# HoangChuongNguyen/ibgs

Measured on AMD Instinct MI355X. Metric: train-step fps (fwd+bwd raster) @1080p, 1M Gaussians, higher is better.
Workload: dtype f32

## Files before the change

ibgs_amd/_build.py:

```python
import os
import subprocess
import sys
from concurrent.futures import ThreadPoolExecutor

HERE = os.path.dirname(os.path.abspath(__file__))
CSRC = os.path.join(HERE, "csrc")
OBJ = os.path.join(CSRC, "_obj")
LIB = os.path.join(HERE, "libibgs_rast.so")
SOURCES = ["api", "preprocess", "scan_sort", "binning", "render_fwd", "render_bwd", "preprocess_bwd", "knn", "adam", "compact", "deterministic", "loss", "depth_normal", "activate"]
EXTRA = {
    "preprocess": ["-ffp-contract=off"],
    "render_fwd": ["-fno-slp-vectorize"],
    "render_bwd": ["-fno-slp-vectorize", "-fno-signed-zeros"],
}
ARCH = "gfx950"


def _hipcc():
    for c in (os.environ.get("HIPCC"), "/opt/rocm/bin/hipcc", "hipcc"):
        if c and (os.path.isabs(c) and os.path.exists(c) or not os.path.isabs(c)):
            return c
    return "hipcc"


def _newest_dep():
    deps = [os.path.join(CSRC, f) for f in os.listdir(CSRC) if f.endswith((".h", ".hip"))]
    deps.append(os.path.join(HERE, "..", "include", "ibgs_rast.h"))
    return max(os.path.getmtime(d) for d in deps)


def _code_only(text):
    import re
    text = re.sub(r"/\*.*?\*/", "", text, flags=re.S)
    text = re.sub(r"//[^\n]*", "", text)
    return "\n".join(l.rstrip() for l in text.split("\n") if l.strip())


def csrc_sha():
    import hashlib
    h = hashlib.sha1()
    for f in sorted(os.listdir(CSRC)):
        if f.endswith((".hip", ".h")):
            h.update(f.encode())
            h.update(_code_only(open(os.path.join(CSRC, f), "r").read()).encode())
    h.update(_code_only(open(os.path.join(HERE, "..", "include", "ibgs_rast.h"), "r").read()).encode())
    return h.hexdigest()[:12]


KERNEL_TU = (("render_fwd", "render_fwd"), ("pack_rgba", "render_fwd"), ("render_bwd", "render_bwd"), ("geo_window", "render_bwd"), ("tile_order", "render_bwd"),
             ("preprocess_bwd", "preprocess_bwd"), ("sh_grad", "preprocess_bwd"), ("preprocess_kernel", "preprocess"), ("sh_color", "preprocess"), ("mark_visible", "preprocess"),
             ("onesweep", "scan_sort"), ("radix", "scan_sort"), ("scan_", "scan_sort"), ("cell_", "binning"), ("expand_", "binning"), ("tile_ranges", "binning"),
             ("rendered_note", "api"), ("l1_", "loss"), ("depth_normal", "depth_normal"), ("activate_", "activate"), ("adam", "adam"), ("compact", "compact"), ("det_", "deterministic"), ("knn", "knn"))


def tu_of(kernel_name):
    for sub, tu in KERNEL_TU:
        if sub in kernel_name:
            return tu
    return None


def tu_shas():
    import hashlib
    hdr = hashlib.sha1()
    for f in sorted(os.listdir(CSRC)):
        if f.endswith(".h"):
            hdr.update(f.encode()); hdr.update(_code_only(open(os.path.join(CSRC, f), "r").read()).encode())
    hdr.update(_code_only(open(os.path.join(HERE, "..", "include", "ibgs_rast.h"), "r").read()).encode())
    out = {}
    for name in SOURCES:
        h = hdr.copy()
        h.update(_code_only(open(os.path.join(CSRC, name + ".hip"), "r").read()).encode())
        h.update(" ".join(EXTRA.get(name, [])).encode())
        out[name] = h.hexdigest()[:12]
    return out


def needs_build():
    if not os.path.exists(LIB):
        return True
    newest = _newest_dep()
    objs = [os.path.join(OBJ, n + ".o") for n in SOURCES]
    return any((not os.path.exists(o)) or os.path.getmtime(o) < newest for o in objs) or os.path.getmtime(LIB) < newest


def build(force=False, verbose=False):
    os.makedirs(OBJ, exist_ok=True)
    hipcc = _hipcc()
    hdr_time = max([os.path.getmtime(os.path.join(CSRC, f)) for f in os.listdir(CSRC) if f.endswith(".h")]
                   + [os.path.getmtime(os.path.join(HERE, "..", "include", "ibgs_rast.h"))])

    def compile_one(name):
        src = os.path.join(CSRC, name + ".hip")
        obj = os.path.join(OBJ, name + ".o")
        if (not force) and os.path.exists(obj) and os.path.getmtime(obj) >= max(os.path.getmtime(src), hdr_time):
            return obj
        cmd = [hipcc, "--offload-arch=" + ARCH, "-O3", "-fPIC", "-std=c++17", "-c", src, "-o", obj] + EXTRA.get(name, [])
        if verbose:
            print(" ".join(cmd), file=sys.stderr)
        subprocess.check_call(cmd)
        return obj

    with ThreadPoolExecutor(max_workers=4) as ex:
        objs = list(ex.map(compile_one, SOURCES))
    if force or (not os.path.exists(LIB)) or os.path.getmtime(LIB) < max(os.path.getmtime(o) for o in objs):
        cmd = [hipcc, "--offload-arch=" + ARCH, "-shared", "-fPIC", "-o", LIB] + objs
        if verbose:
            print(" ".join(cmd), file=sys.stderr)
        subprocess.check_call(cmd)
    return LIB


if __name__ == "__main__":
    print(build(force="--force" in sys.argv, verbose=True))
```

ibgs_amd/csrc/api.hip:

```cpp
#include "common.h"
#include <sched.h>
#include <time.h>
#include <string.h>
#include <cstdlib>
#include <stdlib.h>
#include <stdio.h>
#include <cstdarg>
#include <cstdio>
#include <cstring>
#include <vector>
#include <map>
#include <mutex>

namespace ibgs {

static thread_local char g_err[512] = "";
void set_error(const char* fmt, ...)
{
    va_list ap; va_start(ap, fmt);
    vsnprintf(g_err, sizeof(g_err), fmt, ap);
    va_end(ap);
}

static uint32_t higher_msb(uint32_t n)
{
    uint32_t msb = sizeof(n) * 4, step = msb;
    while (step > 1) {
        step /= 2;
        if (n >> msb) msb += step; else msb -= step;
    }
    if (n >> msb) msb++;
    return msb;
}

GeomState GeomState::carve(char* base, size_t P, size_t* total)
{
    Carver c(base);
    GeomState g;
    g.rec = c.take<float>(P * REC_FLOATS);
    g.depths = c.take<float>(P);
    g.cov3D = c.take<float>(P * 6);
    g.tiles = c.take<uint32_t>(P);
    g.fp = c.take<uint4>(P);
    g.tmask_hi = c.take<uint64_t>(P * (IBGS_CULL_WORDS - 1));
    g.fp_sorted = c.take<uint4>(P);
    g.clamped = c.take<uint8_t>(P);
    g.alive64 = c.take<uint64_t>((P + 63) / 64);
    g.tile_partial = c.take<uint32_t>((P + 63) / 64 + IBGS_MAX_VIEWS + 1);
    g.sort_key[0] = c.take<uint32_t>(P); g.sort_key[1] = c.take<uint32_t>(P);
    g.sort_val[0] = c.take<uint32_t>(P); g.sort_val[1] = c.take<uint32_t>(P);
    g.offsets = c.take<uint32_t>(P + 5);
    g.hist_elems = radix_hist_elems(P);
    g.hist = c.take<uint32_t>(g.hist_elems);
    if (total) *total = (size_t)(c.cur - reinterpret_cast<uintptr_t>(base)) + 128;
    return g;
}

ImgState ImgState::carve(char* base, int W, int H, size_t* total)
{
    Carver c(base);
    ImgState im;
    const size_t HW = (size_t)W * H;
    const size_t tiles = (size_t)((W + TILE - 1) / TILE) * ((H + TILE - 1) / TILE);
    im.ranges = c.take<uint32_t>(tiles * 2);
    im.final_T = c.take<float>(HW);
    im.n_contrib = c.take<uint32_t>(HW);
    im.sum_w = c.take<float>(HW);
    im.low_high = c.take<uint32_t>(HW * 2);
    im.valid_idx = c.take<int32_t>(HW * IBGS_MAX_SRC);
    im.valid_w = c.take<float>(HW * IBGS_MAX_SRC);
    im.meta = c.take<uint32_t>(32);
    im.slot_c = c.take<uint32_t>(HW * IBGS_MAX_BUFFER_LENGTH);
    im.tile_walked = c.take<uint32_t>(tiles * 4);
    im.tile_order = c.take<uint32_t>((tiles + ORDER_CLASSES - 1) / ORDER_CLASSES * ORDER_CLASSES);
    im.tile_risky = c.take<uint32_t>(tiles * 4);
    if (total) *total = (size_t)(c.cur - reinterpret_cast<uintptr_t>(base)) + 128;
    return im;
}

BinState BinState::carve(char* base, size_t R, int W, int H, size_t* total)
{
    Carver c(base);
    BinState b;
    const size_t gx = (size_t)((W + TILE - 1) / TILE), gy = (size_t)((H + TILE - 1) / TILE), ntiles = gx * gy;
    const size_t ncells = ((gx + BIN_CELL - 1) / BIN_CELL) * ((gy + BIN_CELL - 1) / BIN_CELL);
    b.point_list = c.take<uint32_t>(R);
    b.ccap = R;
    b.cent = c.take<uint4>(R);
    b.cnt_elems = (R / 4 > (size_t)65536 ? R / 4 : (size_t)65536) + ncells;
    b.cnt = c.take<uint32_t>(b.cnt_elems);
    b.cell_total = c.take<uint32_t>(ncells);
    b.cell_start = c.take<uint32_t>(ncells + 1);
    b.cell_chunk0 = c.take<uint32_t>(ncells + 1);
    b.chunk_cnt = c.take<uint32_t>((R / BIN_XCHUNK + ncells + 1) * 64);
    b.tile_total = c.take<uint32_t>(ntiles + 1);
    b.scan_elems = scan_scratch_elems(ntiles + 1);
    b.scan_scratch = c.take<uint32_t>(b.scan_elems);
    if (total) *total = (size_t)(c.cur - reinterpret_cast<uintptr_t>(base)) + 128;
    return b;
}

struct TimedPair { hipEvent_t a, b; int stage; };
static uint32_t g_time_mask = 0;
static std::vector<TimedPair> g_pairs;
static std::vector<hipEvent_t> g_free_events;

static hipEvent_t get_event()
{
    if (!g_free_events.empty()) { hipEvent_t e = g_free_events.back(); g_free_events.pop_back(); return e; }
    hipEvent_t e = nullptr;
    (void)hipEventCreate(&e);
    return e;
}

StageTimer::StageTimer(hipStream_t s_, int stage_) : s(s_), stage(stage_), on((g_time_mask >> stage_) & 1u)
{
    if (on) { a = get_event(); b = get_event(); (void)hipEventRecord(a, s); }
}
StageTimer::~StageTimer()
{
    if (on) { (void)hipEventRecord(b, s); g_pairs.push_back({a, b, stage}); }
}

static int stage_check(hipStream_t s, bool debug, const char* what)
{
    if (!debug) return 0;
    hipError_t e = hipStreamSynchronize(s);
    if (e == hipSuccess) e = hipGetLastError();
    if (e != hipSuccess) { set_error("stage '%s' failed: %s", what, hipGetErrorString(e)); return -IBGS_ERR_HIP; }
    return 0;
}

__global__ void __launch_bounds__(1024) rendered_note_kernel(RenderedNote n)
{
    __shared__ unsigned long long s_w[16];
    rendered_note_block<1024>(n, s_w);
}

}

using namespace ibgs;

extern "C" {

const char* ibgs_last_error(void) { return g_err; }
const char* ibgs_version(void) { return "ibgs_rast 0.1 (gfx950)"; }
void ibgs_timing_enable(uint32_t stage_mask) { g_time_mask = stage_mask; }
int32_t ibgs_timing_collect(float* ms, int32_t* launches)
{
    for (int i = 0; i < IBGS_NUM_STAGES; i++) { if (ms) ms[i] = 0.f; if (launches) launches[i] = 0; }
    for (auto& p : g_pairs) {
        float t = 0.f;
        hipError_t e = hipEventSynchronize(p.b);
        if (e == hipSuccess) e = hipEventElapsedTime(&t, p.a, p.b);
        if (e != hipSuccess) { set_error("timing collect: %s", hipGetErrorString(e)); return -IBGS_ERR_HIP; }
        if (ms) ms[p.stage] += t;
        if (launches) launches[p.stage] += 1;
        g_free_events.push_back(p.a); g_free_events.push_back(p.b);
    }
    g_pairs.clear();
    return 0;
}
size_t ibgs_sizeof_forward_args(void) { return sizeof(ibgs_forward_args); }
size_t ibgs_sizeof_backward_args(void) { return sizeof(ibgs_backward_args); }

size_t ibgs_required_geom(int32_t P) { size_t t; GeomState::carve(nullptr, (size_t)(P > 0 ? P : 0), &t); return t; }
size_t ibgs_required_img(int32_t W, int32_t H) { size_t t; ImgState::carve(nullptr, W, H, &t); return t; }
size_t ibgs_required_binning(int64_t R, int32_t W, int32_t H) { size_t t; BinState::carve(nullptr, (size_t)(R > 0 ? R : 0), W, H, &t); return t; }
size_t ibgs_required_deterministic(int64_t R, int32_t P) { size_t t; DetState::carve(nullptr, (size_t)(R > 0 ? R : 0) * 4, (size_t)(P > 0 ? P : 0), &t); return t; }
size_t ibgs_required_tex(int32_t n_src, int32_t W, int32_t H) { return (size_t)n_src * W * H * sizeof(float4) + 128; }
size_t ibgs_required_geo_table(int32_t W, int32_t H) { return geo_table_floats(W, H) * sizeof(float) + 128; }
size_t ibgs_required_geo_table_for(int32_t W, int32_t H, int32_t L)
{
    const int slots = (L >= 1 && L < IBGS_MAX_BUFFER_LENGTH) ? L + 1 : IBGS_MAX_BUFFER_LENGTH;
    return (size_t)W * H * slots * GEO_TAB_FIELDS * sizeof(float) + 128;
}
size_t ibgs_required_deterministic_for(int64_t R, int32_t P, int32_t W, int32_t H, int32_t render_geo, uint32_t flags)
{
    ibgs_backward_args a{}; a.W = W; a.H = H; a.render_geo = render_geo; a.flags = flags;
    size_t t; DetState::carve(nullptr, (size_t)(R > 0 ? R : 0) * render_backward_waves_per_tile(a), (size_t)(P > 0 ? P : 0), &t); return t;
}

#define OFF(base_struct, field) if (!strcmp(name, #field)) return (int64_t)((char*)base_struct.field - (char*)nullptr)
int64_t ibgs_geom_offset(int32_t P, const char* name)
{
    size_t t; GeomState g = GeomState::carve(nullptr, (size_t)P, &t);
    OFF(g, rec); OFF(g, depths); OFF(g, cov3D); OFF(g, tiles); OFF(g, fp); OFF(g, tmask_hi); OFF(g, clamped); OFF(g, offsets);
    if (!strcmp(name, "order")) return (int64_t)((char*)g.sort_val[0] - (char*)nullptr);
    if (!strcmp(name, "order_alt")) return (int64_t)((char*)g.sort_val[1] - (char*)nullptr);
    if (!strcmp(name, "sorted_depth_keys")) return (int64_t)((char*)g.sort_key[0] - (char*)nullptr);
    if (!strcmp(name, "sorted_depth_keys_alt")) return (int64_t)((char*)g.sort_key[1] - (char*)nullptr);
    return -1;
}
size_t ibgs_tile_order_slots(int32_t W, int32_t H)
{
    const size_t tiles = (size_t)((W + TILE - 1) / TILE) * ((H + TILE - 1) / TILE);
    return (tiles + ORDER_CLASSES - 1) / ORDER_CLASSES * ORDER_CLASSES;
}
int64_t ibgs_img_offset(int32_t W, int32_t H, const char* name)
{
    size_t t; ImgState im = ImgState::carve(nullptr, W, H, &t);
    OFF(im, ranges); OFF(im, final_T); OFF(im, n_contrib); OFF(im, sum_w); OFF(im, low_high); OFF(im, valid_idx); OFF(im, valid_w); OFF(im, slot_c); OFF(im, meta); OFF(im, tile_walked); OFF(im, tile_order); OFF(im, tile_risky);
    return -1;
}
int64_t ibgs_binning_offset(int64_t R, int32_t W, int32_t H, const char* name)
{
    size_t t; BinState b = BinState::carve(nullptr, (size_t)R, W, H, &t);
    OFF(b, point_list);
    return -1;
}
#undef OFF

struct RSlot {
    uint32_t* host; hipEvent_t ev;
    uint32_t* stats; bool stats_pending;
    bool flag_pending;
    hipStream_t last_stream;
    uint32_t seq;
};
static std::mutex g_slot_mutex;
static std::map<std::pair<int, hipStream_t>, RSlot*> g_slots;
static RSlot* rslot(hipStream_t s, bool create)
{
    int dev = 0;
    if (hipGetDevice(&dev) != hipSuccess) { set_error("hipGetDevice failed"); return nullptr; }
    std::lock_guard<std::mutex> lock(g_slot_mutex);
    auto it = g_slots.find({dev, s});
    if (it != g_slots.end()) return it->second;
    if (!create) return nullptr;
    RSlot* slot = new RSlot();
    void* p = nullptr;
    if (hipHostMalloc(&p, 64, hipHostMallocCoherent | hipHostMallocMapped) != hipSuccess) { delete slot; set_error("hipHostMalloc for the R read-back failed"); return nullptr; }
    if (hipEventCreateWithFlags(&slot->ev, hipEventDisableTiming) != hipSuccess) { (void)hipHostFree(p); delete slot; set_error("hipEventCreate failed"); return nullptr; }
    slot->host = static_cast<uint32_t*>(p);
    memset(p, 0, 64);
    slot->stats = slot->host + 8;
    slot->stats_pending = false; slot->flag_pending = false; slot->last_stream = s; slot->seq = 0;
    g_slots[{dev, s}] = slot;
    return slot;
}
static int check_sort_flag(RSlot* rs, bool wait_for_note)
{
    if (!rs || !rs->flag_pending) return 0;
    volatile uint32_t* note = rs->stats + 4;
    bool final_ = __atomic_load_n(const_cast<uint32_t*>(note), __ATOMIC_ACQUIRE) == rs->seq;
    if (!final_ && wait_for_note) {
        struct timespec t0, t1; clock_gettime(CLOCK_MONOTONIC, &t0);
        for (uint32_t spins = 1; !final_; spins++) {
            final_ = __atomic_load_n(const_cast<uint32_t*>(note), __ATOMIC_ACQUIRE) == rs->seq;
            if ((spins & 255u) == 0) {
                clock_gettime(CLOCK_MONOTONIC, &t1);
                if ((t1.tv_sec - t0.tv_sec) * 1000000000ll + (t1.tv_nsec - t0.tv_nsec) > 2000000ll) break;
            }
        }
    }
    if (*(volatile uint32_t*)(rs->stats + 3)) {
        rs->stats[3] = 0u; rs->flag_pending = false;
        set_error("depth sort: decoupled look-back timed out (the lists of this stream's last forward were mis-ordered)"); return -IBGS_ERR_HIP;
    }
    if (final_) rs->flag_pending = false;
    return 0;
}

static thread_local int64_t g_last_stats[3] = {0, -1, 0};
static thread_local RSlot* g_stats_slot = nullptr;
void ibgs_last_forward_stats(int64_t* out)
{
    if (g_stats_slot && g_stats_slot->stats_pending) {
        if (hipStreamSynchronize(g_stats_slot->last_stream) == hipSuccess) g_last_stats[1] = (int64_t)*(volatile uint32_t*)(g_stats_slot->stats + 2);
        g_stats_slot->stats_pending = false;
    }
    out[0] = g_last_stats[0]; out[1] = g_last_stats[1]; out[2] = g_last_stats[2];
}
void ibgs_debug_set_lookback_spins(uint32_t v) { radix_set_lookback_spins(v); }
int32_t ibgs_check_async(void* stream, int32_t wait)
{
    hipStream_t s = reinterpret_cast<hipStream_t>(stream);
    RSlot* rs = rslot(s, false);
    if (!rs || !rs->flag_pending) return 0;
    if (wait) IBGS_HIP(hipStreamSynchronize(s));
    return check_sort_flag(rs, false);
}

int64_t ibgs_forward(const ibgs_forward_args* ap)
{
    if (!ap) { set_error("null args"); return -IBGS_ERR_INVALID; }
    const ibgs_forward_args& a = *ap;
    hipStream_t s = reinterpret_cast<hipStream_t>(a.stream);
    const bool debug = (a.flags & IBGS_FLAG_DEBUG) != 0;
    if (a.P < 0 || a.W <= 0 || a.H <= 0) { set_error("bad sizes P=%d W=%d H=%d", a.P, a.W, a.H); return -IBGS_ERR_INVALID; }
    if (a.P == 0) return 0;
    if (!a.means3D || !a.opacities || !a.viewmatrix || !a.projmatrix || !a.campos || !a.bg || !a.radii) {
        set_error("missing required pointer"); return -IBGS_ERR_INVALID;
    }
    if ((a.shs == nullptr) == (a.colors_precomp == nullptr) && !a.render_depth_only) {
        set_error("provide exactly one of shs / colors_precomp"); return -IBGS_ERR_INVALID;
    }
    if (((a.scales == nullptr) || (a.rotations == nullptr)) == (a.cov3D_precomp == nullptr)) {
        set_error("provide exactly one of scales+rotations / cov3D_precomp"); return -IBGS_ERR_INVALID;
    }
    if (a.shs && (a.D < 0 || a.D > 3 || (a.D + 1) * (a.D + 1) > a.M)) { set_error("bad SH degree D=%d M=%d", a.D, a.M); return -IBGS_ERR_INVALID; }
    if (a.shs && a.M == 16 && (reinterpret_cast<uintptr_t>(a.shs) & 15u)) { set_error("shs (M = 16) must be 16-byte aligned"); return -IBGS_ERR_INVALID; }
    if (a.shs_rest && (!a.shs || a.M < 2 || (reinterpret_cast<uintptr_t>(a.shs_rest) & 15u) || (reinterpret_cast<uintptr_t>(a.shs) & 15u))) {
        set_error("shs_rest needs shs (the DC coefficients), M >= 2 and 16-byte aligned arrays"); return -IBGS_ERR_INVALID;
    }
    if (a.render_geo && a.render_depth_only) { set_error("render_geo together with render_depth_only is not supported"); return -IBGS_ERR_INVALID; }
    if (a.plane_mode != IBGS_PLANE_NONE) {
        if (a.all_map) { set_error("give either all_map or plane_mode, not both"); return -IBGS_ERR_INVALID; }
        if (a.plane_mode == IBGS_PLANE_LEARNT ? !a.plane_normal : (a.plane_mode != IBGS_PLANE_SMALLEST_AXIS || !a.scales || !a.rotations)) {
            set_error("plane_mode %d: plane_normal (learnt) or scales + rotations (smallest axis) required", a.plane_mode); return -IBGS_ERR_INVALID;
        }
    }
    if ((a.render_geo || a.render_depth_only) && !a.all_map && a.plane_mode == IBGS_PLANE_NONE) { set_error("all_map (or plane_mode) is required for render_geo / render_depth_only"); return -IBGS_ERR_INVALID; }
    if (a.render_geo || a.render_depth_only) {
        if (a.buffer_length < 1 || a.buffer_length > IBGS_MAX_BUFFER_LENGTH) { set_error("buffer_length %d outside 1..%d", a.buffer_length, IBGS_MAX_BUFFER_LENGTH); return -IBGS_ERR_INVALID; }
        if (!a.out_depth) { set_error("out_depth required"); return -IBGS_ERR_INVALID; }
    }
    if (a.render_geo) {
        if (a.n_src < 1 || a.n_src > IBGS_MAX_SRC) { set_error("n_src %d outside 1..%d", a.n_src, IBGS_MAX_SRC); return -IBGS_ERR_INVALID; }
        if (!a.ref_to_src || !a.src_cam_pos || !a.src_images || !a.src_depths) { set_error("source view pointers required for render_geo"); return -IBGS_ERR_INVALID; }
        if (a.flags & IBGS_FLAG_SRC_DEPTH_SLOTS) {
            for (int m = 0; m < a.n_src; m++) if (a.src_depth_slot[m] < 0) { set_error("src_depth_slot[%d] = %d is negative", m, a.src_depth_slot[m]); return -IBGS_ERR_INVALID; }
        }
        if (!a.out_normal || !a.out_cam_feat || !a.out_warped || !a.out_min_depth_diff || !a.out_camera_ray || !a.out_mask) { set_error("geo outputs required"); return -IBGS_ERR_INVALID; }
        if (!a.tex || a.tex_bytes < ibgs_required_tex(a.n_src, a.W, a.H)) { set_error("tex scratch too small"); return -IBGS_ERR_ALLOC; }
    }
    if (!a.render_depth_only && !a.out_color) { set_error("out_color required"); return -IBGS_ERR_INVALID; }
    const int nv = a.n_views > 1 ? a.n_views : 1;
    if (nv > 1) {
        if (nv > IBGS_MAX_VIEWS || !a.render_depth_only || a.plane_mode == IBGS_PLANE_NONE) {
            set_error("n_views = %d needs render_depth_only, plane_mode != 0 and n_views <= %d", a.n_views, IBGS_MAX_VIEWS); return -IBGS_ERR_INVALID;
        }
        if ((int64_t)nv * a.P > 0x7FFFFFFF) { set_error("n_views x P too large"); return -IBGS_ERR_INVALID; }
    }
    const int Pn = nv * a.P;
    const int Hn = nv > 1 ? nv * TILE * ((a.H + TILE - 1) / TILE) : a.H;
    if (!a.geom || a.geom_bytes < ibgs_required_geom(Pn)) { set_error("geom arena too small"); return -IBGS_ERR_ALLOC; }
    if (!a.img || a.img_bytes < ibgs_required_img(a.W, Hn)) { set_error("img arena too small"); return -IBGS_ERR_ALLOC; }
    if (!a.binning_alloc) { set_error("binning_alloc callback required"); return -IBGS_ERR_INVALID; }

    int rc;
    GeomState g = GeomState::carve(a.geom, (size_t)Pn, nullptr);
    ImgState im = ImgState::carve(a.img, a.W, Hn, nullptr);
    const int gx = (a.W + TILE - 1) / TILE, gy = nv * ((a.H + TILE - 1) / TILE);

    const bool deferred = a.rendered_hint > 0 && !debug;
    const size_t nwaves = (size_t)nv * (((size_t)a.P + 63) / 64);
    RSlot* rs = rslot(s, true);
    if (!rs) return -IBGS_ERR_HIP;
    uint32_t ticket = 0;
    { StageTimer t(s, IBGS_STAGE_PREPROCESS);
      if ((rc = launch_preprocess(s, a, g, deferred ? 1 : 0))) return rc;
      if (deferred) {
          ticket = ++rs->seq;
          const RenderedNote note{g.tile_partial, (uint32_t)nwaves, ticket, rs->host};
          if ((rc = launch_preprocess(s, a, g, 2, &note)) < 0) return rc;
          if (rc == 0) { hipLaunchKernelGGL(rendered_note_kernel, dim3(1), dim3(1024), 0, s, note); IBGS_HIP(hipGetLastError()); }
      }
    }
    if ((rc = stage_check(s, debug, "preprocess"))) return rc;
    { StageTimer t(s, IBGS_STAGE_DEPTH_SORT);
      if ((rc = radix_sort_pairs(s, g.sort_key, g.sort_val, (size_t)Pn, 32, g.hist, g.hist_elems, deferred ? g.tile_partial + nwaves : g.offsets + Pn + 1,
                                 g.offsets + Pn + 3, true, g.offsets + Pn + 4))) return rc; }
    if ((rc = stage_check(s, debug, "depth sort"))) return rc;
    { StageTimer t(s, IBGS_STAGE_SCAN);
      if (!deferred && (rc = exclusive_scan_u32(s, g.tiles, g.offsets, (size_t)Pn, g.hist, g.hist_elems, true))) return rc; }
    auto exact_R = [&](int64_t* R_out) -> int {
        IBGS_HIP(hipMemcpyAsync(rs->host, g.offsets + Pn, 2 * sizeof(uint32_t), hipMemcpyDeviceToHost, s));
        IBGS_HIP(hipEventRecord(rs->ev, s));
        IBGS_HIP(hipEventSynchronize(rs->ev));
        if (rs->host[1]) { set_error("depth sort: decoupled look-back timed out (lists would be mis-ordered)"); return -IBGS_ERR_HIP; }
        *R_out = (int64_t)rs->host[0];
        return 0;
    };
    int64_t R = 0, cap = 0;
    if (deferred) cap = a.rendered_hint < (int64_t)0xFFFF0000ll ? a.rendered_hint : (int64_t)0xFFFF0000ll;
    else { if ((rc = exact_R(&R))) return rc; cap = R; }

    auto tail = [&](int64_t n, bool read_back) -> int {
        int rc;
        const size_t need = ibgs_required_binning(n, a.W, Hn);
        char* bin_mem = (read_back && a.binning && a.binning_bytes >= need) ? a.binning : a.binning_alloc(need, a.binning_user);
        if (!bin_mem) { set_error("binning_alloc returned NULL for R=%lld", (long long)n); return -IBGS_ERR_ALLOC; }
        BinState b = BinState::carve(bin_mem, (size_t)n, a.W, Hn, nullptr);
        { StageTimer t(s, IBGS_STAGE_EMIT);
          if ((rc = launch_binning(s, Pn, n, gx, gy, g, b, im.ranges, a.tile_order_hint, im.meta, nv, read_back ? g.tile_partial + nwaves : nullptr, read_back ? rs->stats : nullptr, ticket))) return rc; }
        if (read_back) { rs->flag_pending = true; rs->last_stream = s; }
        { StageTimer t(s, IBGS_STAGE_TILE_SORT); if ((rc = launch_binning_scatter(s, n, gx, gy, b))) return rc; }
        if ((rc = stage_check(s, debug, "binning"))) return rc;
        const float4* rgba = nullptr;
        if (a.render_geo) {
            float4* t = reinterpret_cast<float4*>((reinterpret_cast<uintptr_t>(a.tex) + 127) & ~uintptr_t(127));
            if (!(a.flags & IBGS_FLAG_TEX_PACKED) && (rc = launch_pack_rgba(s, a.src_images, t, a.W, a.H, a.n_src))) return rc;
            rgba = t;
        }
        { StageTimer t(s, IBGS_STAGE_RENDER_FWD); if ((rc = launch_render_forward(s, a, g, b, im, rgba))) return rc; }
        return stage_check(s, debug, "render");
    };
    const bool prev_pending = rs->flag_pending;
    if ((rc = tail(cap, deferred))) return rc;
    g_last_stats[1] = -1; g_last_stats[2] = 0;
    g_stats_slot = rs; rs->stats_pending = false;
    if (deferred) {
        {
            volatile uint32_t* tk = rs->host + 2;
            const uint32_t want = ticket;
            uint64_t spins = 0;
            struct timespec t0; bool timed = false;
            while (__atomic_load_n(const_cast<uint32_t*>(tk), __ATOMIC_ACQUIRE) != want) {
                if (++spins > 4000) {
                    if (!timed) { clock_gettime(CLOCK_MONOTONIC, &t0); timed = true; }
                    sched_yield();
                    if ((spins & 1023) == 0) {
                        struct timespec t1; clock_gettime(CLOCK_MONOTONIC, &t1);
                        if (t1.tv_sec - t0.tv_sec > 5) {
                            if (hipStreamQuery(s) == hipErrorNotReady) { t0 = t1; continue; }
                            IBGS_HIP(hipStreamSynchronize(s));
                            if (*tk == want) break;
                            set_error("ibgs_forward: the device never reported R (ticket %u, last seen %u)", want, *tk); return -IBGS_ERR_HIP;
                        }
                    }
                }
            }
        }
        if (prev_pending && *(volatile uint32_t*)(rs->stats + 3)) {
            rs->stats[3] = 0u;
            set_error("depth sort of the previous forward: decoupled look-back timed out (its lists were mis-ordered)"); return -IBGS_ERR_HIP;
        }
        const uint64_t sum = (uint64_t)rs->host[0] | ((uint64_t)rs->host[1] << 32);
        R = (int64_t)sum;
        if (R > cap) {
            g_last_stats[2] = 1;
            IBGS_HIP(hipStreamSynchronize(s));
            if ((rc = check_sort_flag(rs, false))) return rc;
            if ((rc = tail(R, false))) return rc;
        } else rs->stats_pending = true;
    }
    g_last_stats[0] = R;
    return R;
}

int32_t ibgs_backward(const ibgs_backward_args* ap)
{
    if (!ap) { set_error("null args"); return -IBGS_ERR_INVALID; }
    const ibgs_backward_args& a = *ap;
    hipStream_t s = reinterpret_cast<hipStream_t>(a.stream);
    const bool debug = (a.flags & IBGS_FLAG_DEBUG) != 0;
    if (a.P <= 0) return 0;
    RSlot* rs = rslot(s, false);
    { int frc = check_sort_flag(rs, false); if (frc) return frc; }
    if (!a.geom || !a.img || (!a.binning && a.R > 0)) { set_error("backward needs the forward's arenas"); return -IBGS_ERR_INVALID; }
    if (!a.grad_acc) { set_error("grad_acc scratch required"); return -IBGS_ERR_INVALID; }
    if (!a.dL_dmean2D || (!a.dL_dmean2D_abs && !(a.flags & IBGS_FLAG_NO_ABS_GRAD)) || !a.dL_dopacity || !a.dL_dmean3D) {
        set_error("missing gradient output"); return -IBGS_ERR_INVALID;
    }
    if (a.shs && !a.dL_dsh && !(a.flags & IBGS_FLAG_SH_FACTORED)) { set_error("dL_dsh required"); return -IBGS_ERR_INVALID; }
    if (a.shs_rest && (!a.shs || a.M < 2 || (!(a.flags & IBGS_FLAG_SH_FACTORED) && !a.dL_dsh_rest)
                       || ((reinterpret_cast<uintptr_t>(a.shs_rest) | reinterpret_cast<uintptr_t>(a.shs) | reinterpret_cast<uintptr_t>(a.dL_dsh_rest) | reinterpret_cast<uintptr_t>(a.dL_dsh)) & 15u))) {
        set_error("shs_rest needs shs, M >= 2, dL_dsh_rest and 16-byte aligned arrays"); return -IBGS_ERR_INVALID;
    }
    if (a.shs && a.M == 16 && ((reinterpret_cast<uintptr_t>(a.shs) & 15u) || (a.dL_dsh && (reinterpret_cast<uintptr_t>(a.dL_dsh) & 15u)))) {
        set_error("shs / dL_dsh (M = 16) must be 16-byte aligned"); return -IBGS_ERR_INVALID;
    }
    if (!a.dL_dcolors && (!a.shs || (a.flags & IBGS_FLAG_SH_FACTORED))) { set_error("dL_dcolors required (precomputed colours, or IBGS_FLAG_SH_FACTORED)"); return -IBGS_ERR_INVALID; }
    if (!a.dL_dcov3D && a.cov3D_precomp) { set_error("dL_dcov3D required with cov3D_precomp"); return -IBGS_ERR_INVALID; }
    if (a.scales && (!a.dL_dscale || !a.dL_drot)) { set_error("dL_dscale / dL_drot required"); return -IBGS_ERR_INVALID; }
    if (a.render_geo) {
        if (a.plane_mode == IBGS_PLANE_NONE ? (!a.all_map || !a.dL_dall_map)
                                            : (a.plane_mode == IBGS_PLANE_LEARNT ? (!a.plane_normal || !a.dL_dplane_normal)
                                                                                 : (a.plane_mode != IBGS_PLANE_SMALLEST_AXIS || !a.scales || !a.rotations))) {
            set_error("geo backward: plane inputs / gradient outputs missing"); return -IBGS_ERR_INVALID;
        }
        if (!a.out_depth || !a.out_warped || !a.ref_to_src || !a.src_images) { set_error("geo backward inputs missing"); return -IBGS_ERR_INVALID; }
        if (!a.tex || a.tex_bytes < ibgs_required_tex(a.n_src, a.W, a.H)) { set_error("tex scratch too small"); return -IBGS_ERR_ALLOC; }
        if (!a.geo_table || a.geo_table_bytes < (a.buffer_length > 0 ? ibgs_required_geo_table_for(a.W, a.H, a.buffer_length) : ibgs_required_geo_table(a.W, a.H))) { set_error("geo_table scratch too small"); return -IBGS_ERR_ALLOC; }
    }
    int rc;
    GeomState g = GeomState::carve(a.geom, (size_t)a.P, nullptr);
    ImgState im = ImgState::carve(a.img, a.W, a.H, nullptr);
    BinState b = BinState::carve(a.binning, (size_t)a.R, a.W, a.H, nullptr);
    const float4* rgba = nullptr;
    float* geo_tab = nullptr;
    if (a.render_geo) {
        float4* t = reinterpret_cast<float4*>((reinterpret_cast<uintptr_t>(a.tex) + 127) & ~uintptr_t(127));
        const bool window = a.dL_ddepth || a.dL_dwarped;
        if (window && !(a.flags & IBGS_FLAG_TEX_PACKED) && (rc = launch_pack_rgba(s, a.src_images, t, a.W, a.H, a.n_src))) return rc;
        rgba = t;
        geo_tab = reinterpret_cast<float*>((reinterpret_cast<uintptr_t>(a.geo_table) + 127) & ~uintptr_t(127));
    }
    if (a.R > 0) {
        const bool det = (a.flags & IBGS_FLAG_DETERMINISTIC) != 0;
        DetState ds{};
        int ipt = 1;
        if (det) {
            if (!a.det_scratch || a.det_scratch_bytes < ibgs_required_deterministic_for(a.R, a.P, a.W, a.H, a.render_geo, a.flags)) { set_error("det_scratch too small"); return -IBGS_ERR_ALLOC; }
            ipt = render_backward_waves_per_tile(a);
            ds = DetState::carve(a.det_scratch, (size_t)a.R * ipt, (size_t)a.P, nullptr);
            if ((rc = launch_det_prepare(s, ds, (size_t)a.R * ipt))) return rc;
        }
        if ((rc = launch_render_backward(s, a, g, b, im, rgba, det ? ds.slab : nullptr, geo_tab))) return rc;
        if (det) { StageTimer t(s, IBGS_STAGE_TILE_ORDER); if ((rc = launch_det_reduce(s, ds, b.point_list, (size_t)a.R, ipt, a.P, a.grad_acc, g.offsets + a.P))) return rc; }
        if ((rc = stage_check(s, debug, "render backward"))) return rc;
    }
    { StageTimer t(s, IBGS_STAGE_PREPROCESS_BWD); if ((rc = launch_preprocess_backward(s, a, g))) return rc; }
    if ((rc = stage_check(s, debug, "preprocess backward"))) return rc;
    return check_sort_flag(rs, true);
}

int32_t ibgs_sh_grad_from_views(void* stream, int32_t P, int32_t D, int32_t M, int32_t n_views, const float* means3D,
                                const float* camposes, const float* dcolor, int64_t view_stride, float* dL_dsh)
{
    if (view_stride == 0) view_stride = (int64_t)P * 3;
    if (view_stride < (int64_t)P * 3) { set_error("view_stride smaller than P x 3"); return -IBGS_ERR_INVALID; }
    if (P <= 0 || M <= 0) return 0;
    if (D < 0 || D > 3 || (D + 1) * (D + 1) > M || n_views < 0) { set_error("bad SH degree / view count"); return -IBGS_ERR_INVALID; }
    if (!means3D || !dL_dsh || (n_views > 0 && (!camposes || !dcolor))) { set_error("null pointer"); return -IBGS_ERR_INVALID; }
    return launch_sh_grad_from_views(reinterpret_cast<hipStream_t>(stream), P, D, M, n_views, means3D, camposes, dcolor, (size_t)view_stride, dL_dsh);
}

int32_t ibgs_mark_visible(void* stream, int32_t P, const float* means3D, const float* viewmatrix,
                          const float* projmatrix, uint8_t* present)
{
    (void)projmatrix;
    if (P <= 0) return 0;
    if (!means3D || !viewmatrix || !present) { set_error("null pointer"); return -IBGS_ERR_INVALID; }
    return launch_mark_visible(reinterpret_cast<hipStream_t>(stream), P, means3D, viewmatrix, present);
}

}
```

ibgs_amd/csrc/common.h:

```cpp
#pragma once
#include <hip/hip_runtime.h>
#include <stdint.h>
#include <stddef.h>
#include <stdlib.h>
#include "../../include/ibgs_rast.h"

namespace ibgs {

constexpr int TILE = IBGS_TILE;
constexpr int WAVE = 64;
constexpr int REC_FLOATS = 16;
constexpr int GACC_FLOATS = 16;

constexpr int IBGS_CULL_WORDS = 4;
constexpr int IBGS_CULL_MAX_TILES = 64 * IBGS_CULL_WORDS;

enum RecField { R_X = 0, R_Y = 1, R_OP = 2, R_PAD0 = 3, R_CA = 4, R_CB = 5, R_CC = 6, R_DIST = 7,
                R_R = 8, R_G = 9, R_B = 10, R_PAD1 = 11, R_NX = 12, R_NY = 13, R_NZ = 14, R_PAD2 = 15 };

enum GaccField { G_SX = 0, G_SY = 1, G_AX = 2, G_AY = 3, G_SXX = 4, G_SXY = 5, G_SYY = 6, G_S0 = 7,
                 G_R = 8, G_G = 9, G_B = 10, G_NX = 11, G_NY = 12, G_NZ = 13, G_DIST = 14, G_PAD = 15 };

struct Carver {
    uintptr_t cur;
    explicit Carver(char* base) : cur(reinterpret_cast<uintptr_t>(base)) {}
    template <typename T> T* take(size_t count) {
        cur = (cur + 127) & ~uintptr_t(127);
        T* p = reinterpret_cast<T*>(cur);
        cur += count * sizeof(T);
        return p;
    }
};

struct GeomState {
    float* rec;
    float* depths;
    float* cov3D;
    uint32_t* tiles;
    uint4* fp;
    uint64_t* tmask_hi;
    uint4* fp_sorted;
    uint8_t* clamped;
    uint64_t* alive64;
    uint32_t* tile_partial;
    uint32_t* sort_key[2];
    uint32_t* sort_val[2];
    uint32_t* offsets;
    uint32_t* hist;
    size_t hist_elems;
    static GeomState carve(char* base, size_t P, size_t* total);
};

struct ImgState {
    uint32_t* ranges;
    float* final_T;
    uint32_t* n_contrib;
    float* sum_w;
    uint32_t* low_high;
    int32_t* valid_idx;
    float* valid_w;
    uint32_t* meta;
    uint32_t* slot_c;
    uint32_t* tile_walked;
    uint32_t* tile_order;
    uint32_t* tile_risky;
    static ImgState carve(char* base, int W, int H, size_t* total);
};

constexpr int BIN_CELL = 8;
constexpr int BIN_XCHUNK = 256;

struct BinState {
    uint32_t* point_list;
    uint4* cent;
    uint32_t* cnt;
    size_t cnt_elems;
    uint32_t* cell_total;
    uint32_t* cell_start;
    uint32_t* cell_chunk0;
    uint32_t* chunk_cnt;
    uint32_t* tile_total;
    uint32_t* scan_scratch; size_t scan_elems;
    size_t ccap;
    static BinState carve(char* base, size_t R, int W, int H, size_t* total);
};

constexpr float EXP2_SCALE = 0.5f * 1.4426950408889634f;
constexpr float EXP2_UNSCALE = 1.0f / EXP2_SCALE;
constexpr float ALPHA_SKIP_E = 7.9943533f;
__device__ __forceinline__ void stage_for_exp2(float4& pos_opacity_quad, float4& conic_quad)
{
    conic_quad.x *= EXP2_SCALE; conic_quad.y *= EXP2_SCALE; conic_quad.z *= EXP2_SCALE;
    pos_opacity_quad.z = -__builtin_amdgcn_logf(pos_opacity_quad.z);
}

constexpr float POWER_RISK = 0.99999f;
constexpr float LOG2_E = 1.4426950408889634f;
__device__ __forceinline__ bool conic_is_risky(float a, float b, float c) { return b * b > POWER_RISK * (a * c); }
constexpr float BLEND_REF_POWER_RISK = 0.999f;
__device__ __forceinline__ bool conic_takes_ref_power(float a, float b, float c) { return b * b > BLEND_REF_POWER_RISK * (a * c); }
__device__ __forceinline__ float ref_power_E(float dx, float dy, float a, float b, float c, float neg_log2_opacity)
{
#pragma clang fp contract(off)
    const float power = -0.5f * (a * dx * dx + c * dy * dy) - b * dx * dy;
    return power > 0.0f ? __builtin_inff() : fmaf(-power, LOG2_E, neg_log2_opacity);
}

__device__ __forceinline__ float ln_portable(float x)
{
#pragma clang fp contract(off)
    uint32_t u = __float_as_uint(x);
    const int e = (int)(u >> 23) - 127;
    u = (u & 0x007FFFFFu) | 0x3F800000u;
    const float m = __uint_as_float(u);
    const float s = (m - 1.0f) / (m + 1.0f), z = s * s;
    const float poly = 1.0f + z * (0.33333334f + z * (0.2f + z * (0.14285715f + z * 0.11111111f)));
    return (float)e * 0.6931472f + 2.0f * s * poly;
}
__device__ __forceinline__ float cull_qmax(float o)
{
#pragma clang fp contract(off)
    return 2.0f * ln_portable(255.0f * o) * 1.001f + 0.001f;
}
struct CullRows { float px, py, B, det, invA, aq, ymax, ystar; int x0, x1; };
__device__ __forceinline__ void cull_rows_setup(CullRows& j, float px, float py, float A, float B, float C, float det, float qmax, int x0, int x1)
{
#pragma clang fp contract(off)
    j.px = px; j.py = py; j.B = B; j.det = det; j.x0 = x0; j.x1 = x1;
    j.invA = 1.0f / A; j.aq = A * qmax;
    j.ymax = sqrtf(j.aq / det); j.ystar = -B * sqrtf(qmax / (C * det));
}
__device__ __forceinline__ void cull_rows_setup_conic(CullRows& j, float px, float py, float A, float B, float C, float qmax, int x0, int x1)
{
#pragma clang fp contract(off)
    const float det = A * C - B * B;
    cull_rows_setup(j, px, py, A, B, C, det, qmax, x0, x1);
}
__device__ __forceinline__ bool cull_row_run(const CullRows& j, int ty, int& t0, int& t1)
{
#pragma clang fp contract(off)
    const float Y0 = (float)(ty * 16) - j.py, Y1 = Y0 + 15.0f;
    const float yb0 = Y0 > -j.ymax ? Y0 : -j.ymax, yb1 = Y1 < j.ymax ? Y1 : j.ymax;
    if (yb0 > yb1) return false;
    const float yu = __builtin_amdgcn_fmed3f(j.ystar, yb0, yb1), yl = __builtin_amdgcn_fmed3f(-j.ystar, yb0, yb1);
    const float eu = j.aq - j.det * yu * yu, el = j.aq - j.det * yl * yl;
    const float du = eu > 0.0f ? eu : 0.0f, dl = el > 0.0f ? el : 0.0f;
    const float xhi = (-j.B * yu + sqrtf(du)) * j.invA, xlo = (-j.B * yl - sqrtf(dl)) * j.invA;
    t0 = (int)ceilf((xlo - 0.01f + j.px - 15.0f) / 16.0f); t1 = (int)floorf((xhi + 0.01f + j.px) / 16.0f);
    t0 = max(t0, j.x0); t1 = min(t1, j.x1 - 1);
    return t1 >= t0;
}

#ifdef IBGS_TRACE_WAVES
constexpr int IBGS_TRACE_MAX = 32768;
#define IBGS_TRACE_BEGIN() const unsigned long long ibgs_trace_t0_ = __builtin_amdgcn_s_memrealtime()
#define IBGS_TRACE_END(buf)                                                                                         \
    do {                                                                                                            \
        const unsigned long long t1_ = __builtin_amdgcn_s_memrealtime();                                            \
        if (threadIdx.x == 0 && blockIdx.x < (unsigned)IBGS_TRACE_MAX)                                              \
            (buf)[blockIdx.x] = make_uint4(__builtin_amdgcn_s_getreg((31 << 11) | 4), __builtin_amdgcn_s_getreg((31 << 11) | 20), \
                                           (uint32_t)ibgs_trace_t0_, (uint32_t)t1_);                                \
    } while (0)
#else
#define IBGS_TRACE_BEGIN() do { } while (0)
#define IBGS_TRACE_END(buf) do { } while (0)
#endif

#ifdef IBGS_COUNT_LANES
#define IBGS_LANES_DECL() unsigned long long ibgs_lc_[4] = {0ull, 0ull, 0ull, 0ull}
#define IBGS_LANES_ADD(i, n) ibgs_lc_[i] += (unsigned long long)(n)
#define IBGS_LANES_FLUSH(buf) do { if (threadIdx.x == 0) { for (int i_ = 0; i_ < 4; i_++) atomicAdd(&(buf)[i_], ibgs_lc_[i_]); } } while (0)
#else
#define IBGS_LANES_DECL() do { } while (0)
#define IBGS_LANES_ADD(i, n) do { } while (0)
#define IBGS_LANES_FLUSH(buf) do { } while (0)
#endif

void set_error(const char* fmt, ...);
#define IBGS_HIP(expr)                                                                    \
    do {                                                                                  \
        hipError_t e_ = (expr);                                                           \
        if (e_ != hipSuccess) {                                                           \
            ::ibgs::set_error("%s failed: %s (%s:%d)", #expr, hipGetErrorString(e_), __FILE__, __LINE__); \
            return -IBGS_ERR_HIP;                                                         \
        }                                                                                 \
    } while (0)

struct StageTimer {
    hipStream_t s; hipEvent_t a = nullptr, b = nullptr; int stage; bool on;
    StageTimer(hipStream_t s_, int stage_);
    ~StageTimer();
};

struct Cam {
    const float* vm;
    const float* pm;
    const float* campos;
    const float* bg;
    float tanfovx, tanfovy, fx, fy;
    int W, H, gx, gy;
};
inline Cam make_cam(const float* vm, const float* pm, const float* campos, const float* bg,
                    float tanfovx, float tanfovy, int W, int H)
{
    Cam c;
    c.vm = vm; c.pm = pm; c.campos = campos; c.bg = bg;
    c.tanfovx = tanfovx; c.tanfovy = tanfovy;
    c.fy = H / (2.0f * tanfovy); c.fx = W / (2.0f * tanfovx);
    c.W = W; c.H = H; c.gx = (W + TILE - 1) / TILE; c.gy = (H + TILE - 1) / TILE;
    return c;
}


struct PlaneEval {
    float n[3];
    float ncam[3];
    float dist;
    float flip;
    float sgn;
    float inv_len;
    int axis;
};

__device__ __forceinline__ PlaneEval plane_eval(int mode, const float* __restrict__ raw_n, const float* __restrict__ raw_off,
                                                const float* __restrict__ scales, const float* __restrict__ rot, int i,
                                                float mx, float my, float mz, const float* __restrict__ campos,
                                                const float* __restrict__ vm)
{
    PlaneEval e;
    float off = 0.f;
    e.inv_len = 1.f; e.axis = 0;
    if (mode == IBGS_PLANE_LEARNT) {
        const float a = raw_n[3 * i], b = raw_n[3 * i + 1], c = raw_n[3 * i + 2];
        const float len = sqrtf(a * a + b * b + c * c);
        e.inv_len = 1.0f / len;
        e.n[0] = a / len; e.n[1] = b / len; e.n[2] = c / len;
        off = raw_off ? raw_off[i] : 0.f;
    } else {
        const float s0 = scales[3 * i], s1 = scales[3 * i + 1], s2 = scales[3 * i + 2];
        int k = 0; float sm = s0;
        if (s1 < sm) { sm = s1; k = 1; }
        if (s2 < sm) { sm = s2; k = 2; }
        e.axis = k;
        const float r = rot[4 * i], x = rot[4 * i + 1], y = rot[4 * i + 2], z = rot[4 * i + 3];
        if (k == 0)      { e.n[0] = 1.f - 2.f * (y * y + z * z); e.n[1] = 2.f * (x * y + r * z);       e.n[2] = 2.f * (x * z - r * y); }
        else if (k == 1) { e.n[0] = 2.f * (x * y - r * z);       e.n[1] = 1.f - 2.f * (x * x + z * z); e.n[2] = 2.f * (y * z + r * x); }
        else             { e.n[0] = 2.f * (x * z + r * y);       e.n[1] = 2.f * (y * z - r * x);       e.n[2] = 1.f - 2.f * (x * x + y * y); }
    }
    const float tc = e.n[0] * (campos[0] - mx) + e.n[1] * (campos[1] - my) + e.n[2] * (campos[2] - mz);
    e.flip = (tc < 0.0f) ? -1.f : 1.f;
    e.n[0] *= e.flip; e.n[1] *= e.flip; e.n[2] *= e.flip; off *= e.flip;
#pragma unroll
    for (int j = 0; j < 3; j++) e.ncam[j] = e.n[0] * vm[j] + e.n[1] * vm[4 + j] + e.n[2] * vm[8 + j];
    float gd = -(e.n[0] * mx + e.n[1] * my + e.n[2] * mz);
    if (mode == IBGS_PLANE_LEARNT) gd += off;
    const float sd = gd - (e.ncam[0] * vm[12] + e.ncam[1] * vm[13] + e.ncam[2] * vm[14]);
    e.sgn = sd > 0.f ? 1.f : (sd < 0.f ? -1.f : 0.f);
    e.dist = fabsf(sd);
    return e;
}

enum { TMAP_RR = 0, TMAP_GROUP = 1, TMAP_BLOCK = 2 };
struct TileMap { int mode, g, bx, by; };
inline int tile_map_grid(const TileMap& m, int gx, int gy, int ipt)
{
    if (m.mode == TMAP_BLOCK) {
        const int nb = ((gx + m.bx - 1) / m.bx) * ((gy + m.by - 1) / m.by);
        return ((nb + 7) / 8) * 8 * m.bx * m.by * ipt;
    }
    const int g = m.mode == TMAP_GROUP ? m.g : 1;
    return ((gx * gy * ipt + 8 * g - 1) / (8 * g)) * 8 * g;
}
__device__ __forceinline__ bool tile_map_item(const TileMap& m, int b, int gx, int gy, int ipt, int& tile, int& sub)
{
    const int xcd = b & 7, idx = b >> 3;
    if (m.mode == TMAP_BLOCK) {
        const int per = m.bx * m.by * ipt;
        const int blk = (idx / per) * 8 + xcd, within = idx % per;
        const int nbx = (gx + m.bx - 1) / m.bx;
        const int t = within / ipt;
        const int tx = (blk % nbx) * m.bx + t % m.bx, ty = (blk / nbx) * m.by + t / m.bx;
        sub = within % ipt;
        tile = ty * gx + tx;
        return tx < gx && ty < gy;
    }
    int item = b;
    if (m.mode == TMAP_GROUP) item = ((idx / m.g) * 8 + xcd) * m.g + idx % m.g;
    tile = item / ipt; sub = item % ipt;
    return item < gx * gy * ipt;
}

__device__ __forceinline__ bool hybrid_split(uint32_t work, unsigned long long total, uint32_t theta_pct)
{
    return (unsigned long long)work * 1024ull * 100ull > total * theta_pct;
}
constexpr uint32_t ORDER_SPLIT_BIT = 0x80000000u;
__device__ __forceinline__ bool hybrid_item(int b, int grid1, const uint32_t* __restrict__ order, int& tile, int& sub, bool& split)
{
    const int idx = (b - grid1) >> 3;
    const int slot = b < grid1 ? b : (idx / 3) * 8 + (b & 7);
    sub = b < grid1 ? 0 : idx % 3 + 1;
    const uint32_t t = order[slot];
    split = (t & ORDER_SPLIT_BIT) != 0u;
    tile = (int)(t & ~ORDER_SPLIT_BIT);
    return t != 0xFFFFFFFFu;
}
__device__ __forceinline__ bool hybrid_item_mapped(const TileMap& m, int b, int grid1, int gx, int gy, int& tile, int& sub)
{
    if (b < grid1) { const bool ok = tile_map_item(m, b, gx, gy, 1, tile, sub); sub = 0; return ok; }
    const bool ok = tile_map_item(m, b - grid1, gx, gy, 3, tile, sub);
    sub += 1;
    return ok;
}
constexpr int HYBRID_THETA = 50;
constexpr int HYBRID_MIN_TILES = 768;
constexpr int hybrid_max_tiles() { return 4096; }
constexpr int hybrid_theta() { return HYBRID_THETA; }

struct RenderedNote { const uint32_t* partial; uint32_t nwords; uint32_t ticket; uint32_t* host; };
template <int NT>
__device__ __forceinline__ void rendered_note_block(const RenderedNote& n, unsigned long long* s_w )
{
    unsigned long long sum = 0;
    for (uint32_t i = threadIdx.x; i < n.nwords; i += NT) sum += n.partial[i];
    for (int d = 32; d >= 1; d >>= 1) sum += __shfl_xor(sum, d, 64);
    if ((threadIdx.x & 63) == 0) s_w[threadIdx.x >> 6] = sum;
    __syncthreads();
    if (threadIdx.x == 0) {
        unsigned long long t = 0;
        for (int w = 0; w < NT / 64; w++) t += s_w[w];
        volatile uint32_t* host_words = n.host;
        host_words[0] = (uint32_t)t; host_words[1] = (uint32_t)(t >> 32);
        __threadfence_system();
        __hip_atomic_store(n.host + 2, n.ticket, __ATOMIC_RELEASE, __HIP_MEMORY_SCOPE_SYSTEM);
    }
}
int launch_preprocess(hipStream_t s, const ibgs_forward_args& a, const GeomState& g, int phase = 0, const RenderedNote* note = nullptr);
int launch_mark_visible(hipStream_t s, int P, const float* means3D, const float* vm, uint8_t* present);

size_t radix_hist_elems(size_t n);
int radix_sort_pairs(hipStream_t s, uint32_t* keys[2], uint32_t* vals[2], size_t n, int nbits,
                     uint32_t* hist, size_t hist_elems, uint32_t* err_dev = nullptr, uint32_t* kept_dev = nullptr, bool scratch_is_zero = false,
                     uint32_t* result_alt = nullptr);
size_t radix_zero_elems(size_t n, int nbits);
int exclusive_scan_u32(hipStream_t s, const uint32_t* in, uint32_t* out, size_t n, uint32_t* scratch,
                       size_t scratch_elems, bool with_total);
size_t scan_scratch_elems(size_t n);
void radix_set_onesweep(bool on);
void radix_set_lookback_spins(uint32_t v);

int launch_binning(hipStream_t s, int P, int64_t cap, int gx, int gy, const GeomState& g, const BinState& b, uint32_t* ranges,
                   const uint32_t* order_hint = nullptr, uint32_t* meta = nullptr ,
                   int n_views = 1 ,
                   const uint32_t* sort_flag = nullptr, uint32_t* host_note = nullptr ,
                   uint32_t note_ticket = 0 );
constexpr int ORDER_CLASSES = 1024;
int launch_binning_scatter(hipStream_t s, int64_t cap, int gx, int gy, const BinState& b);

int launch_pack_rgba(hipStream_t s, const float* src, float4* dst, int W, int H, int n);
constexpr int GEO_TAB_FIELDS = 6;
inline size_t geo_table_floats(int W, int H) { return (size_t)W * H * IBGS_MAX_BUFFER_LENGTH * GEO_TAB_FIELDS; }
int launch_render_forward(hipStream_t s, const ibgs_forward_args& a, const GeomState& g, const BinState& b,
                          const ImgState& im, const float4* src_rgba);
int launch_render_backward(hipStream_t s, const ibgs_backward_args& a, const GeomState& g, const BinState& b,
                           const ImgState& im, const float4* src_rgba, float* slab = nullptr, float* geo_tab = nullptr);
int launch_preprocess_backward(hipStream_t s, const ibgs_backward_args& a, const GeomState& g);

struct DetState {
    float* slab;
    uint32_t* keys[2];
    uint32_t* vals[2];
    uint32_t* seg;
    uint32_t* hist; size_t hist_elems;
    static DetState carve(char* base, size_t rows, size_t P, size_t* total);
};
int render_backward_waves_per_tile(const ibgs_backward_args& a);
int render_backward_ref_arith(uint32_t flags);
int launch_det_prepare(hipStream_t s, const DetState& d, size_t rows);
int launch_det_reduce(hipStream_t s, const DetState& d, const uint32_t* point_list, size_t R, int ipt, int P, float* gacc, const uint32_t* listed );
int launch_sh_grad_from_views(hipStream_t s, int P, int D, int M, int n_views, const float* means3D, const float* camposes,
                              const float* dcolor, size_t view_stride, float* dL_dsh);

__device__ __forceinline__ uint32_t pack_rect(int lo, int hi) { return (uint32_t)lo | ((uint32_t)hi << 16); }

}
```

ibgs_amd/csrc/preprocess.hip:

```cpp
#include "common.h"
#include <stdlib.h>

namespace ibgs {

__constant__ float kC0 = 0.28209479177387814f;
__constant__ float kC1 = 0.4886025119029199f;
__constant__ float kC2[5] = {1.0925484305920792f, -1.0925484305920792f, 0.31539156525252005f,
                             -1.0925484305920792f, 0.5462742152960396f};
__constant__ float kC3[7] = {-0.5900435899266435f, 2.890611442640554f, -0.4570457994644658f,
                             0.3731763325901154f, -0.4570457994644658f, 1.445305721320277f,
                             -0.5900435899266435f};

struct PreParams {
    int P, D, M;
    const float* means3D; const float* scales; const float* rotations; const float* opacities;
    const float* shs; const float* shs_rest;
    const float* cov3D_precomp; const float* colors_precomp; const float* all_map;
    const float* plane_normal; const float* plane_offset; int plane_mode;
    int inst0;
    int tile_row0;
    float scale_modifier;
    int depth_only;
    int32_t* radii;
    float* rec; float* depths; float* cov3D; uint32_t* tiles; uint4* fp; uint64_t* tmask_hi; uint8_t* clamped;
    uint64_t* alive64;
    uint32_t* sort_key; uint32_t* sort_val;
    int cull;
    uint32_t* zero_a; uint32_t zero_a_n; uint32_t* zero_b; uint32_t zero_b_n;
    RenderedNote note;
    uint32_t* tile_partial; int partial0; int partial_err;
};

__device__ __forceinline__ float ndc_to_pix(float v, int S)
{
    return (float)((((double)v + 1.0) * S - 1.0) * 0.5);
}

__device__ __forceinline__ int clampi(int v, int lo, int hi) { return min(hi, max(lo, v)); }

struct CullJob { CullRows rows; int y0, w, h; };
enum { CULL_NONE = 0, CULL_AABB = 1, CULL_ROWS = 2 };

__device__ __forceinline__ int cull_setup(float px, float py, float sxx, float syy, float A, float B, float C, float o,
                                          int& x0, int& y0, int& x1, int& y1, CullJob& j)
{
    if (conic_is_risky(A, B, C)) return CULL_AABB;
    const float x255 = 255.0f * o;
    if (!(x255 >= 1.0f)) { x1 = x0; y1 = y0; return CULL_NONE; }
    const float qmax = cull_qmax(o);
    const float hx = sqrtf(qmax * sxx), hy = sqrtf(qmax * syy);
    int tx0 = (int)ceilf((px - hx - 15.0f) / 16.0f), tx1 = (int)floorf((px + hx) / 16.0f) + 1;
    int ty0 = (int)ceilf((py - hy - 15.0f) / 16.0f), ty1 = (int)floorf((py + hy) / 16.0f) + 1;
    tx0 = max(tx0, x0); tx1 = min(tx1, x1); ty0 = max(ty0, y0); ty1 = min(ty1, y1);
    if (tx1 <= tx0 || ty1 <= ty0) { x1 = x0; y1 = y0; return CULL_NONE; }
    x0 = tx0; x1 = tx1; y0 = ty0; y1 = ty1;
    const float det = A * C - B * B;
    if (!(A > 0.0f) || !(C > 0.0f) || !(det > 0.0f)) return CULL_AABB;
    cull_rows_setup(j.rows, px, py, A, B, C, det, qmax, tx0, tx1);
    j.y0 = ty0; j.w = tx1 - tx0; j.h = ty1 - ty0;
    return CULL_ROWS;
}

__device__ __forceinline__ void set_run(uint64_t (&m)[IBGS_CULL_WORDS], int start, int len)
{
#pragma unroll
    for (int k = 0; k < IBGS_CULL_WORDS; k++) {
        const int lo = max(start, 64 * k), hi = min(start + len, 64 * k + 64);
        if (lo < hi) m[k] |= ((hi - lo == 64) ? ~0ull : ((1ull << (hi - lo)) - 1ull)) << (lo - 64 * k);
    }
}

constexpr int CULL_COOP_ROWS = 16;
__device__ __forceinline__ void park_job(float4* stage_row, const CullJob& j)
{
    stage_row[0] = make_float4(j.rows.px, j.rows.py, j.rows.B, j.rows.det);
    stage_row[1] = make_float4(j.rows.invA, j.rows.aq, j.rows.ymax, j.rows.ystar);
    stage_row[2] = make_float4(__uint_as_float((uint32_t)j.rows.x0 | ((uint32_t)j.rows.x1 << 16)), __uint_as_float((uint32_t)j.y0 | ((uint32_t)j.h << 16)), 0.f, 0.f);
    stage_row[3] = make_float4(0.f, 0.f, 0.f, 0.f);
    stage_row[4] = make_float4(0.f, 0.f, 0.f, 0.f);
}
__device__ __forceinline__ void fetch_job(const float4* stage_row, CullJob& j)
{
    const float4 q0 = stage_row[0], q1 = stage_row[1], q2 = stage_row[2];
    j.rows.px = q0.x; j.rows.py = q0.y; j.rows.B = q0.z; j.rows.det = q0.w;
    j.rows.invA = q1.x; j.rows.aq = q1.y; j.rows.ymax = q1.z; j.rows.ystar = q1.w;
    const uint32_t xs = __float_as_uint(q2.x), ys = __float_as_uint(q2.y);
    j.rows.x0 = (int)(xs & 0xFFFFu); j.rows.x1 = (int)(xs >> 16);
    j.y0 = (int)(ys & 0xFFFFu); j.h = (int)(ys >> 16); j.w = j.rows.x1 - j.rows.x0;
}
__device__ __forceinline__ void wave_flat_rows(float4* stage, int rows, int lane)
{
    uint32_t* words = reinterpret_cast<uint32_t*>(stage);
    int incl = rows;
#pragma unroll
    for (int d = 1; d < 64; d <<= 1) { const int o = __shfl_up(incl, d, 64); if (lane >= d) incl += o; }
    const int total = __builtin_amdgcn_readlane(incl, 63);
    for (int base = 0; base < total; base += 64) {
        const int item = base + lane;
        int lo = 0;
#pragma unroll
        for (int step = 32; step >= 1; step >>= 1) { const int v = __shfl(incl, lo + step - 1, 64); if (v <= item) lo += step; }
        const int owner = min(lo, 63);
        const int r = item - (__shfl(incl, owner, 64) - __shfl(rows, owner, 64));
        if (item < total) {
            CullJob u;
            fetch_job(stage + owner * 5, u);
            int t0, t1;
            if (cull_row_run(u.rows, u.y0 + r, t0, t1)) {
                uint32_t* ow = words + owner * 20;
                atomicAdd(ow + 10, (uint32_t)(t1 - t0 + 1));
                if (u.w * u.h <= IBGS_CULL_MAX_TILES) {
                    const int s0 = r * u.w + (t0 - u.rows.x0), e0 = s0 + (t1 - t0 + 1);
                    for (int k = s0 >> 5; k <= (e0 - 1) >> 5; k++) {
                        const int lo_b = max(s0, 32 * k) - 32 * k, hi_b = min(e0, 32 * k + 32) - 32 * k;
                        atomicOr(ow + 12 + k, ((hi_b - lo_b == 32) ? ~0u : ((1u << (hi_b - lo_b)) - 1u)) << lo_b);
                    }
                }
            }
        }
    }
}

template <bool WITH_SH>
__global__ void __launch_bounds__(256, 4) preprocess_kernel(PreParams p, Cam cam)
{
    __shared__ float4 s_stage_all[4][64 * 5];
    float4* s_stage = s_stage_all[threadIdx.x >> 6];
    const int gi = blockIdx.x * blockDim.x + threadIdx.x;
    for (uint32_t z = (uint32_t)gi; z < p.zero_a_n; z += gridDim.x * blockDim.x) p.zero_a[z] = 0u;
    if ((uint32_t)gi < p.zero_b_n) p.zero_b[gi] = 0u;
    const bool valid = gi < p.P;
    const int i = valid ? gi : p.P - 1;

    float rec[REC_FLOATS];
#pragma unroll
    for (int k = 0; k < REC_FLOATS; k++) rec[k] = 0.f;
    int radius = 0; uint32_t ntiles = 0; float depth = 0.f; uint8_t clampbits = 0;
    float c6loc[6] = {0, 0, 0, 0, 0, 0};

    const float px3 = p.means3D[3 * i], py3 = p.means3D[3 * i + 1], pz3 = p.means3D[3 * i + 2];
    const float* __restrict__ vm = cam.vm; const float* __restrict__ pm = cam.pm;
    const float hx = pm[0] * px3 + pm[4] * py3 + pm[8] * pz3 + pm[12];
    const float hy = pm[1] * px3 + pm[5] * py3 + pm[9] * pz3 + pm[13];
    const float hw = pm[3] * px3 + pm[7] * py3 + pm[11] * pz3 + pm[15];
    const float pw = 1.0f / (hw + 0.0000001f);
    const float zview = vm[2] * px3 + vm[6] * py3 + vm[10] * pz3 + vm[14];

    bool alive = zview > 0.2f;
    float ca = 0.f, cb = 0.f, cc = 0.f, det_inv = 0.f, pxs = 0.f, pys = 0.f;
    int x0 = 0, y0 = 0, x1 = 0, y1 = 0;
    int walk_rows = 0;
    bool full_mask = false;
    const int lane = threadIdx.x & 63;
    if (alive) {
        if (p.cov3D_precomp) {
#pragma unroll
            for (int k = 0; k < 6; k++) c6loc[k] = p.cov3D_precomp[6 * i + k];
        } else {
            const float r = p.rotations[4 * i], x = p.rotations[4 * i + 1], y = p.rotations[4 * i + 2], z = p.rotations[4 * i + 3];
            float R[3][3];
            R[0][0] = 1.f - 2.f * (y * y + z * z); R[0][1] = 2.f * (x * y - r * z);       R[0][2] = 2.f * (x * z + r * y);
            R[1][0] = 2.f * (x * y + r * z);       R[1][1] = 1.f - 2.f * (x * x + z * z); R[1][2] = 2.f * (y * z - r * x);
            R[2][0] = 2.f * (x * z - r * y);       R[2][1] = 2.f * (y * z + r * x);       R[2][2] = 1.f - 2.f * (x * x + y * y);
            const float sv[3] = {p.scale_modifier * p.scales[3 * i], p.scale_modifier * p.scales[3 * i + 1],
                                 p.scale_modifier * p.scales[3 * i + 2]};
            float Mm[3][3];
#pragma unroll
            for (int a = 0; a < 3; a++)
#pragma unroll
                for (int b = 0; b < 3; b++) Mm[a][b] = sv[a] * R[b][a];
#define SIG(a, b) (Mm[0][a] * Mm[0][b] + Mm[1][a] * Mm[1][b] + Mm[2][a] * Mm[2][b])
            c6loc[0] = SIG(0, 0); c6loc[1] = SIG(0, 1); c6loc[2] = SIG(0, 2);
            c6loc[3] = SIG(1, 1); c6loc[4] = SIG(1, 2); c6loc[5] = SIG(2, 2);
#undef SIG
        }
        float t0 = vm[0] * px3 + vm[4] * py3 + vm[8] * pz3 + vm[12];
        float t1 = vm[1] * px3 + vm[5] * py3 + vm[9] * pz3 + vm[13];
        const float t2 = vm[2] * px3 + vm[6] * py3 + vm[10] * pz3 + vm[14];
        const float limx = 1.3f * cam.tanfovx, limy = 1.3f * cam.tanfovy;
        const float txtz = t0 / t2, tytz = t1 / t2;
        t0 = fminf(limx, fmaxf(-limx, txtz)) * t2;
        t1 = fminf(limy, fmaxf(-limy, tytz)) * t2;
        const float j00 = cam.fx / t2, j02 = -(cam.fx * t0) / (t2 * t2);
        const float j11 = cam.fy / t2, j12 = -(cam.fy * t1) / (t2 * t2);
        float A[2][3];
#pragma unroll
        for (int r = 0; r < 3; r++) {
            const float rv0 = vm[4 * r + 0], rv1 = vm[4 * r + 1], rv2 = vm[4 * r + 2];
            A[0][r] = rv0 * j00 + rv1 * 0.0f + rv2 * j02;
            A[1][r] = rv0 * 0.0f + rv1 * j11 + rv2 * j12;
        }
        const float S[3][3] = {{c6loc[0], c6loc[1], c6loc[2]}, {c6loc[1], c6loc[3], c6loc[4]}, {c6loc[2], c6loc[4], c6loc[5]}};
        float SA[2][3];
#pragma unroll
        for (int a = 0; a < 2; a++)
#pragma unroll
            for (int r = 0; r < 3; r++) SA[a][r] = S[r][0] * A[a][0] + S[r][1] * A[a][1] + S[r][2] * A[a][2];
        ca = A[0][0] * SA[0][0] + A[0][1] * SA[0][1] + A[0][2] * SA[0][2] + 0.3f;
        cb = A[0][0] * SA[1][0] + A[0][1] * SA[1][1] + A[0][2] * SA[1][2];
        cc = A[1][0] * SA[1][0] + A[1][1] * SA[1][1] + A[1][2] * SA[1][2] + 0.3f;
        const float det = ca * cc - cb * cb;
        alive = (det != 0.0f);
        if (alive) {
            det_inv = 1.f / det;
            const float mid = 0.5f * (ca + cc);
            const float disc = sqrtf(fmaxf(0.1f, mid * mid - det));
            const float lam1 = mid + disc, lam2 = mid - disc;
            const float my_radius = ceilf(3.f * sqrtf(fmaxf(lam1, lam2)));
            pxs = ndc_to_pix(hx * pw, cam.W); pys = ndc_to_pix(hy * pw, cam.H);
            const int rad = (int)my_radius;
            x0 = clampi((int)((pxs - rad) / TILE), 0, cam.gx);
            y0 = clampi((int)((pys - rad) / TILE), 0, cam.gy);
            x1 = clampi((int)((pxs + rad + TILE - 1) / TILE), 0, cam.gx);
            y1 = clampi((int)((pys + rad + TILE - 1) / TILE), 0, cam.gy);
            alive = ((x1 - x0) * (y1 - y0)) != 0;
            if (alive) {
                radius = rad; ntiles = (uint32_t)((x1 - x0) * (y1 - y0));
                full_mask = true;
                if (p.cull) {
                    CullJob job;
                    const int cull_mode = cull_setup(pxs, pys, ca, cc, cc * det_inv, -cb * det_inv, ca * det_inv, p.opacities[i], x0, y0, x1, y1, job);
                    if (cull_mode == CULL_NONE) { ntiles = 0; full_mask = false; }
                    else if (cull_mode == CULL_AABB) ntiles = (uint32_t)((x1 - x0) * (y1 - y0));
                    else {
                        full_mask = false;
                        walk_rows = job.h;
                        park_job(s_stage + lane * 5, job);
                    }
                }
            }
        }
    }
    if (p.cull) {
        const bool tall = walk_rows > CULL_COOP_ROWS;
        if (__ballot(walk_rows != 0) != 0ull) {
            wave_flat_rows(s_stage, tall ? 0 : walk_rows, lane);
            uint64_t todo = __ballot(tall);
            while (todo != 0ull) {
                const int g = __builtin_ctzll(todo);
                todo &= todo - 1ull;
                CullJob u;
                fetch_job(s_stage + g * 5, u);
                const bool masked = u.w * u.h <= IBGS_CULL_MAX_TILES;
                uint64_t m[IBGS_CULL_WORDS] = {0, 0, 0, 0};
                uint32_t cnt = 0;
                for (int r = lane; r < u.h; r += 64) {
                    int t0, t1;
                    if (!cull_row_run(u.rows, u.y0 + r, t0, t1)) continue;
                    if (masked) set_run(m, r * u.w + (t0 - u.rows.x0), t1 - t0 + 1);
                    cnt += (uint32_t)(t1 - t0 + 1);
                }
#pragma unroll
                for (int d = 32; d >= 1; d >>= 1) cnt += (uint32_t)__shfl_xor((int)cnt, d, 64);
                uint32_t* ow = reinterpret_cast<uint32_t*>(s_stage) + g * 20;
                if (masked) {
#pragma unroll
                    for (int k = 0; k < IBGS_CULL_WORDS; k++) {
                        uint32_t lo = (uint32_t)m[k], hi = (uint32_t)(m[k] >> 32);
#pragma unroll
                        for (int d = 32; d >= 1; d >>= 1) { lo |= (uint32_t)__shfl_xor((int)lo, d, 64); hi |= (uint32_t)__shfl_xor((int)hi, d, 64); }
                        if (lane == 0) { ow[12 + 2 * k] = lo; ow[13 + 2 * k] = hi; }
                    }
                }
                if (lane == 0) ow[10] = cnt;
            }
        }
    }
    {
        uint64_t tmask[IBGS_CULL_WORDS];
        const uint32_t* ow = reinterpret_cast<const uint32_t*>(s_stage) + lane * 20;
#pragma unroll
        for (int k = 0; k < IBGS_CULL_WORDS; k++) tmask[k] = walk_rows != 0 ? (((uint64_t)ow[13 + 2 * k] << 32) | ow[12 + 2 * k]) : (full_mask ? ~0ull : 0ull);
        if (walk_rows != 0) ntiles = ow[10];
        uint32_t rx = 0, ry = 0;
        bool big_rect = false;
        if (alive) {
            big_rect = (x1 - x0) * (y1 - y0) > 64 && (x1 - x0) * (y1 - y0) <= IBGS_CULL_MAX_TILES;
            rx = pack_rect(x0, x1); ry = pack_rect(y0 + (uint32_t)p.tile_row0, y1 + (uint32_t)p.tile_row0);
        }
        if (valid) {
            const int o = p.inst0 + i;
            p.fp[o] = make_uint4(rx, ry, (uint32_t)tmask[0], (uint32_t)(tmask[0] >> 32));
            if (big_rect) {
#pragma unroll
                for (int k = 1; k < IBGS_CULL_WORDS; k++) p.tmask_hi[(size_t)o * (IBGS_CULL_WORDS - 1) + (k - 1)] = tmask[k];
            }
        }
    }
    if (alive) {
        depth = zview;
        rec[R_X] = pxs; rec[R_Y] = pys; rec[R_OP] = p.opacities[i];
        rec[R_CA] = cc * det_inv; rec[R_CB] = -cb * det_inv; rec[R_CC] = ca * det_inv;
        if (p.colors_precomp) {
            rec[R_R] = p.colors_precomp[3 * i]; rec[R_G] = p.colors_precomp[3 * i + 1]; rec[R_B] = p.colors_precomp[3 * i + 2];
        } else if (WITH_SH && !p.depth_only) {
            float d0 = px3 - cam.campos[0], d1 = py3 - cam.campos[1], d2 = pz3 - cam.campos[2];
            const float len = sqrtf(d0 * d0 + d1 * d1 + d2 * d2);
            d0 /= len; d1 /= len; d2 /= len;
            float B[16];
            int nb = 1;
            B[0] = kC0;
            if (p.D > 0) {
                const float x = d0, y = d1, z = d2;
                B[1] = -kC1 * y; B[2] = kC1 * z; B[3] = -kC1 * x; nb = 4;
                if (p.D > 1) {
                    const float xx = x * x, yy = y * y, zz = z * z, xy = x * y, yz = y * z, xz = x * z;
                    B[4] = kC2[0] * xy; B[5] = kC2[1] * yz; B[6] = kC2[2] * (2.0f * zz - xx - yy);
                    B[7] = kC2[3] * xz; B[8] = kC2[4] * (xx - yy); nb = 9;
                    if (p.D > 2) {
                        B[9] = kC3[0] * y * (3.0f * xx - yy);
                        B[10] = kC3[1] * xy * z;
                        B[11] = kC3[2] * y * (4.0f * zz - xx - yy);
                        B[12] = kC3[3] * z * (2.0f * zz - 3.0f * xx - 3.0f * yy);
                        B[13] = kC3[4] * x * (4.0f * zz - xx - yy);
                        B[14] = kC3[5] * z * (xx - yy);
                        B[15] = kC3[6] * x * (xx - 3.0f * yy);
                        nb = 16;
                    }
                }
            }
            float shv[48];
            const float* sh = p.shs + (size_t)i * p.M * 3;
            const int need = 3 * nb;
            if (p.shs_rest) {
                const float* sr = p.shs_rest + (size_t)i * (p.M - 1) * 3;
                const float* sd = p.shs + (size_t)i * 3;
#pragma unroll
                for (int k = 0; k < 48; k++) if (k < need) shv[k] = k < 3 ? sd[k] : sr[k - 3];
            } else if (p.M == 16) {
                const float4* r4 = reinterpret_cast<const float4*>(sh);
#pragma unroll
                for (int v = 0; v < 12; v++) {
                    if (4 * v < need) {
                        const float4 q = r4[v];
                        shv[4 * v] = q.x; shv[4 * v + 1] = q.y; shv[4 * v + 2] = q.z; shv[4 * v + 3] = q.w;
                    }
                }
            } else {
#pragma unroll
                for (int k = 0; k < 48; k++) if (k < need) shv[k] = sh[k];
            }
            float col[3];
#pragma unroll
            for (int ch = 0; ch < 3; ch++) col[ch] = B[0] * shv[ch];
#pragma unroll
            for (int k = 1; k < 16; k++) {
                if (k < nb) {
#pragma unroll
                    for (int ch = 0; ch < 3; ch++) col[ch] = col[ch] + B[k] * shv[3 * k + ch];
                }
            }
#pragma unroll
            for (int ch = 0; ch < 3; ch++) {
                const float v = col[ch] + 0.5f;
                if (v < 0) clampbits |= (uint8_t)(1u << ch);
                rec[R_R + ch] = fmaxf(v, 0.0f);
            }
        }
        if (p.plane_mode) {
            const PlaneEval e = plane_eval(p.plane_mode, p.plane_normal, p.plane_offset, p.scales, p.rotations, i, px3, py3, pz3, cam.campos, vm);
            rec[R_NX] = e.ncam[0]; rec[R_NY] = e.ncam[1]; rec[R_NZ] = e.ncam[2]; rec[R_DIST] = e.dist;
        } else if (p.all_map) {
            rec[R_NX] = p.all_map[5 * i]; rec[R_NY] = p.all_map[5 * i + 1]; rec[R_NZ] = p.all_map[5 * i + 2];
            rec[R_DIST] = p.all_map[5 * i + 4];
        }
    }
    if (!alive) {
#pragma unroll
        for (int k = 0; k < REC_FLOATS; k++) rec[k] = 0.f;
    }
    {
#pragma unroll
        for (int k = 0; k < 4; k++) s_stage[lane * 5 + k] = make_float4(rec[4 * k], rec[4 * k + 1], rec[4 * k + 2], rec[4 * k + 3]);
        const int first = blockIdx.x * blockDim.x + (threadIdx.x & ~63);
        const int nrow = min(64, p.P - first);
        float4* out = reinterpret_cast<float4*>(p.rec) + ((size_t)p.inst0 + first) * 4;
#pragma unroll
        for (int it = 0; it < 4; it++) {
            const int q = it * 64 + lane, row = q >> 2;
            if (row < nrow) out[q] = s_stage[row * 5 + (q & 3)];
        }
    }
    if (p.alive64) {
        const uint64_t am = __ballot(valid && alive && ntiles > 0);
        if ((threadIdx.x & 63) == 0) p.alive64[gi >> 6] = am;
    }
    {
        uint32_t tsum = valid ? ntiles : 0u;
#pragma unroll
        for (int d = 32; d >= 1; d >>= 1) tsum += (uint32_t)__shfl_xor((int)tsum, d, 64);
        if ((threadIdx.x & 63) == 0) p.tile_partial[p.partial0 + (gi >> 6)] = tsum;
        if (gi == 0) p.tile_partial[p.partial_err] = 0u;
    }
    if (!valid) return;

    const int o = p.inst0 + i;
    p.radii[o] = radius;
    p.tiles[o] = ntiles;
    p.depths[o] = depth;
    p.clamped[o] = clampbits;
    if (!p.cov3D_precomp) {
#pragma unroll
        for (int k = 0; k < 6; k++) p.cov3D[6 * o + k] = c6loc[k];
    }
    p.sort_key[o] = (alive && ntiles > 0) ? __float_as_uint(depth) : 0xFFFFFFFFu;
    p.sort_val[o] = (uint32_t)o;
}

constexpr int SHC_ROW = 52;
template <bool SPLIT>
__global__ void __launch_bounds__(256) sh_color_kernel(PreParams p, Cam cam)
{
    __shared__ float s_sh_all[4][32 * SHC_ROW];
    if (p.note.host != nullptr && blockIdx.x == 0) {
        __shared__ unsigned long long s_note[4];
        rendered_note_block<256>(p.note, s_note);
    }
    float* s_sh = s_sh_all[threadIdx.x >> 6];
    const int lane = threadIdx.x & 63;
    const int wave = blockIdx.x * 4 + (threadIdx.x >> 6);
    const int first = wave * 64;
    if (first >= p.P) return;
    const uint64_t alive_m = p.alive64[wave];
    if (alive_m == 0ull) return;
    const int i = min(first + lane, p.P - 1);
    const bool alive = (alive_m >> lane) & 1ull;
    const int D = p.D, M = p.M;
    const int nb = (D + 1) * (D + 1);
    const float px3 = p.means3D[3 * i], py3 = p.means3D[3 * i + 1], pz3 = p.means3D[3 * i + 2];
    float shv[48];
    if (SPLIT && M == 16 && first + 64 <= p.P) {
        const float4* rest4 = reinterpret_cast<const float4*>(p.shs_rest + (size_t)first * 45);
        const float4* dc4 = reinterpret_cast<const float4*>(p.shs + (size_t)first * 3);
        float4 v[12];
#pragma unroll
        for (int it = 0; it < 12; it++) {
            const int h = it / 6, qp = (it % 6) * 64 + lane;
            if (qp < 360) {
                const int ra = (4 * qp) / 45, rb = (4 * qp + 3) / 45;
                const bool need = nb > 1 && (((alive_m >> (32 * h + ra)) & 1ull) || ((alive_m >> (32 * h + rb)) & 1ull));
                v[it] = need ? rest4[360 * h + qp] : make_float4(0.f, 0.f, 0.f, 0.f);
            } else {
                const int ra = (4 * (qp - 360)) / 3, rb = (4 * (qp - 360) + 3) / 3;
                const bool need = (((alive_m >> (32 * h + ra)) & 3ull) != 0ull) || ((alive_m >> (32 * h + rb)) & 1ull);
                v[it] = need ? dc4[24 * h + (qp - 360)] : make_float4(0.f, 0.f, 0.f, 0.f);
            }
        }
        float4* s_raw = reinterpret_cast<float4*>(s_sh);
#pragma unroll
        for (int h = 0; h < 2; h++) {
#pragma unroll
            for (int it = 0; it < 6; it++) s_raw[it * 64 + lane] = v[h * 6 + it];
            if ((lane >> 5) == h) {
                const float* rr = s_sh + 45 * (lane & 31);
                const float* rd = s_sh + 1440 + 3 * (lane & 31);
                shv[0] = rd[0]; shv[1] = rd[1]; shv[2] = rd[2];
#pragma unroll
                for (int k = 0; k < 45; k++) shv[3 + k] = rr[k];
            }
        }
    } else if (SPLIT) {
        const float* sr = p.shs_rest + (size_t)i * (M - 1) * 3;
        const float* sd = p.shs + (size_t)i * 3;
#pragma unroll
        for (int k = 0; k < 48; k++) shv[k] = (alive && k < 3 * nb) ? (k < 3 ? sd[k] : sr[k - 3]) : 0.f;
    } else if (M == 16) {
        const float4* src = reinterpret_cast<const float4*>(p.shs) + (size_t)first * 12;
        const int nq = min(64, p.P - first) * 12;
        float4 v[12];
#pragma unroll
        for (int it = 0; it < 12; it++) {
            const int q = it * 64 + lane;
            const int row = q / 12, piece = q - row * 12;
            const bool ok = q < nq && ((alive_m >> row) & 1ull) && 4 * piece < 3 * nb;
            v[it] = ok ? src[q] : make_float4(0.f, 0.f, 0.f, 0.f);
        }
#pragma unroll
        for (int h = 0; h < 2; h++) {
#pragma unroll
            for (int it = 0; it < 6; it++) {
                const int q = it * 64 + lane;
                const int row = q / 12, piece = q - row * 12;
                *reinterpret_cast<float4*>(s_sh + row * SHC_ROW + piece * 4) = v[h * 6 + it];
            }
            if ((lane >> 5) == h) {
                const float4* row4 = reinterpret_cast<const float4*>(s_sh + (lane & 31) * SHC_ROW);
#pragma unroll
                for (int k = 0; k < 12; k++) { const float4 q = row4[k]; shv[4 * k] = q.x; shv[4 * k + 1] = q.y; shv[4 * k + 2] = q.z; shv[4 * k + 3] = q.w; }
            }
        }
    } else {
        const float* sh = p.shs + (size_t)i * M * 3;
#pragma unroll
        for (int k = 0; k < 48; k++) shv[k] = (alive && k < 3 * nb) ? sh[k] : 0.f;
    }
    if (!alive) return;
    float d0 = px3 - cam.campos[0], d1 = py3 - cam.campos[1], d2 = pz3 - cam.campos[2];
    const float len = sqrtf(d0 * d0 + d1 * d1 + d2 * d2);
    d0 /= len; d1 /= len; d2 /= len;
    float B[16];
    B[0] = kC0;
    if (D > 0) {
        const float x = d0, y = d1, z = d2;
        B[1] = -kC1 * y; B[2] = kC1 * z; B[3] = -kC1 * x;
        if (D > 1) {
            const float xx = x * x, yy = y * y, zz = z * z, xy = x * y, yz = y * z, xz = x * z;
            B[4] = kC2[0] * xy; B[5] = kC2[1] * yz; B[6] = kC2[2] * (2.0f * zz - xx - yy);
            B[7] = kC2[3] * xz; B[8] = kC2[4] * (xx - yy);
            if (D > 2) {
                B[9] = kC3[0] * y * (3.0f * xx - yy);
                B[10] = kC3[1] * xy * z;
                B[11] = kC3[2] * y * (4.0f * zz - xx - yy);
                B[12] = kC3[3] * z * (2.0f * zz - 3.0f * xx - 3.0f * yy);
                B[13] = kC3[4] * x * (4.0f * zz - xx - yy);
                B[14] = kC3[5] * z * (xx - yy);
                B[15] = kC3[6] * x * (xx - 3.0f * yy);
            }
        }
    }
    float col[3];
#pragma unroll
    for (int ch = 0; ch < 3; ch++) col[ch] = B[0] * shv[ch];
#pragma unroll
    for (int k = 1; k < 16; k++) {
        if (k < nb) {
#pragma unroll
            for (int ch = 0; ch < 3; ch++) col[ch] = col[ch] + B[k] * shv[3 * k + ch];
        }
    }
    const int o = p.inst0 + i;
    uint8_t clampbits = 0;
    float4 out;
    float* oc = &out.x;
#pragma unroll
    for (int ch = 0; ch < 3; ch++) {
        const float v = col[ch] + 0.5f;
        if (v < 0) clampbits |= (uint8_t)(1u << ch);
        oc[ch] = fmaxf(v, 0.0f);
    }
    out.w = 0.f;
    reinterpret_cast<float4*>(p.rec)[(size_t)o * 4 + 2] = out;
    p.clamped[o] = clampbits;
}

__global__ void __launch_bounds__(256) mark_visible_kernel(int P, const float* means3D, Cam cam, uint8_t* present)
{
    const int i = blockIdx.x * blockDim.x + threadIdx.x;
    if (i >= P) return;
    const float z = cam.vm[2] * means3D[3 * i] + cam.vm[6] * means3D[3 * i + 1] + cam.vm[10] * means3D[3 * i + 2] + cam.vm[14];
    present[i] = z > 0.2f ? 1 : 0;
}

static bool preprocess_is_split(const ibgs_forward_args& a)
{
    return a.shs && !a.colors_precomp && !a.render_depth_only;
}

int launch_preprocess(hipStream_t s, const ibgs_forward_args& a, const GeomState& g, int phase, const RenderedNote* note)
{
    PreParams p;
    p.note = RenderedNote{nullptr, 0u, 0u, nullptr};
    int carried = 0;
    p.P = a.P; p.D = a.D; p.M = a.M;
    p.means3D = a.means3D; p.scales = a.scales; p.rotations = a.rotations; p.opacities = a.opacities;
    p.shs = a.shs; p.shs_rest = a.shs_rest; p.cov3D_precomp = a.cov3D_precomp; p.colors_precomp = a.colors_precomp; p.all_map = a.all_map;
    p.plane_normal = a.plane_normal; p.plane_offset = a.plane_offset; p.plane_mode = a.plane_mode;
    p.scale_modifier = a.scale_modifier; p.depth_only = a.render_depth_only;
    p.radii = a.radii; p.rec = g.rec; p.depths = g.depths; p.cov3D = g.cov3D; p.tiles = g.tiles; p.fp = g.fp; p.tmask_hi = g.tmask_hi;
    p.clamped = g.clamped; p.sort_key = g.sort_key[0]; p.sort_val = g.sort_val[0];
    p.cull = !(a.flags & IBGS_FLAG_NO_TILE_CULL) && !(a.render_depth_only && a.buffer_length == 1);
    const int blocks = (a.P + 255) / 256;
    const int nv = a.n_views > 1 ? a.n_views : 1;
    const int gy = (a.H + TILE - 1) / TILE;
    p.zero_a = g.hist; p.zero_a_n = (uint32_t)radix_zero_elems((size_t)nv * a.P, 32);
    p.zero_b = g.offsets + (size_t)nv * a.P + 1; p.zero_b_n = 4;
    for (int v = 0; v < nv; v++) {
        p.inst0 = v * a.P; p.tile_row0 = v * gy;
        p.tile_partial = g.tile_partial; p.partial0 = v * ((a.P + 63) / 64); p.partial_err = nv * ((a.P + 63) / 64);
        const Cam cam = make_cam(a.viewmatrix + 16 * v, a.projmatrix + 16 * v, a.campos + 3 * v, a.bg,
                                 nv > 1 ? a.view_tanfovx[v] : a.tanfovx, nv > 1 ? a.view_tanfovy[v] : a.tanfovy, a.W, a.H);
        const bool split = preprocess_is_split(a);
        p.alive64 = split ? g.alive64 : nullptr;
        const bool no_sh = a.render_depth_only || a.colors_precomp || !a.shs;
        if (split) {
            if (phase != 2) hipLaunchKernelGGL(preprocess_kernel<false>, dim3(blocks), dim3(256), 0, s, p, cam);
            if (phase != 1) {
                if (note && !carried) { p.note = *note; carried = 1; } else p.note.host = nullptr;
                if (p.shs_rest) hipLaunchKernelGGL(sh_color_kernel<true>, dim3((a.P + 255) / 256), dim3(256), 0, s, p, cam);
                else hipLaunchKernelGGL(sh_color_kernel<false>, dim3((a.P + 255) / 256), dim3(256), 0, s, p, cam);
            }
        } else if (phase != 2) hipLaunchKernelGGL(preprocess_kernel<false>, dim3(blocks), dim3(256), 0, s, p, cam);
    }
    IBGS_HIP(hipGetLastError());
    return carried;
}

int launch_mark_visible(hipStream_t s, int P, const float* means3D, const float* vm, uint8_t* present)
{
    const Cam cam = make_cam(vm, nullptr, nullptr, nullptr, 1.f, 1.f, 16, 16);
    hipLaunchKernelGGL(mark_visible_kernel, dim3((P + 255) / 256), dim3(256), 0, s, P, means3D, cam, present);
    IBGS_HIP(hipGetLastError());
    return 0;
}

}
```

ibgs_amd/csrc/scan_sort.hip:

```cpp
#include "common.h"
#include <cstdlib>

namespace ibgs {

constexpr int SCAN_THREADS = 256;
constexpr int SCAN_ITEMS = 8;
constexpr int SCAN_CHUNK = SCAN_THREADS * SCAN_ITEMS;

constexpr int RS_THREADS = 256;
constexpr int RS_ITEMS = 16;
constexpr int RS_CHUNK = RS_THREADS * RS_ITEMS;
constexpr int RS_MAX_BINS = 256;

__device__ __forceinline__ uint32_t wave_inclusive_scan(uint32_t v, int lane)
{
#pragma unroll
    for (int d = 1; d < WAVE; d <<= 1) {
        const uint32_t o = __shfl_up(v, d, WAVE);
        if (lane >= d) v += o;
    }
    return v;
}

__device__ __forceinline__ uint32_t block_exclusive_scan_256(uint32_t v, uint32_t* total, uint32_t* lds_wave )
{
    const int lane = threadIdx.x & 63, wave = threadIdx.x >> 6;
    const uint32_t inc = wave_inclusive_scan(v, lane);
    if (lane == 63 && wave < 4) lds_wave[wave] = inc;
    __syncthreads();
    const uint32_t w0 = lds_wave[0], w1 = lds_wave[1], w2 = lds_wave[2], w3 = lds_wave[3];
    uint32_t base = 0;
    if (wave > 0) base += w0;
    if (wave > 1) base += w1;
    if (wave > 2) base += w2;
    *total = w0 + w1 + w2 + w3;
    __syncthreads();
    return base + inc - v;
}

__global__ void __launch_bounds__(SCAN_THREADS) scan_chunk_kernel(const uint32_t* in, uint32_t* out,
                                                                  size_t n, uint32_t* __restrict__ sums, int write_total_single)
{
    __shared__ uint32_t lds_wave[4];
    const size_t base = (size_t)blockIdx.x * SCAN_CHUNK + (size_t)threadIdx.x * SCAN_ITEMS;
    uint32_t v[SCAN_ITEMS];
    uint32_t local = 0;
#pragma unroll
    for (int k = 0; k < SCAN_ITEMS; k++) {
        v[k] = (base + k < n) ? in[base + k] : 0u;
        local += v[k];
    }
    uint32_t total;
    uint32_t pre = block_exclusive_scan_256(local, &total, lds_wave);
#pragma unroll
    for (int k = 0; k < SCAN_ITEMS; k++) {
        if (base + k < n) out[base + k] = pre;
        pre += v[k];
    }
    if (threadIdx.x == 0) {
        if (sums) sums[blockIdx.x] = total;
        if (write_total_single) out[n] = total;
    }
}

__global__ void __launch_bounds__(SCAN_THREADS) scan_add_kernel(uint32_t* __restrict__ out, size_t n, const uint32_t* __restrict__ sums,
                                                                size_t nblocks, int write_total)
{
    const size_t base = (size_t)blockIdx.x * SCAN_CHUNK + (size_t)threadIdx.x * SCAN_ITEMS;
    const uint32_t add = sums[blockIdx.x];
#pragma unroll
    for (int k = 0; k < SCAN_ITEMS; k++)
        if (base + k < n) out[base + k] += add;
    if (write_total && blockIdx.x == 0 && threadIdx.x == 0) out[n] = sums[nblocks];
}

size_t scan_scratch_elems(size_t n)
{
    size_t total = 0;
    while (n > SCAN_CHUNK) {
        n = (n + SCAN_CHUNK - 1) / SCAN_CHUNK;
        total += n + 1 + 32;
    }
    return total + 64;
}

int exclusive_scan_u32(hipStream_t s, const uint32_t* in, uint32_t* out, size_t n, uint32_t* scratch,
                       size_t scratch_elems, bool with_total)
{
    if (n == 0) {
        if (with_total) IBGS_HIP(hipMemsetAsync(out, 0, sizeof(uint32_t), s));
        return 0;
    }
    const size_t nblocks = (n + SCAN_CHUNK - 1) / SCAN_CHUNK;
    if (nblocks == 1) {
        hipLaunchKernelGGL(scan_chunk_kernel, dim3(1), dim3(SCAN_THREADS), 0, s, in, out, n, (uint32_t*)nullptr, with_total ? 1 : 0);
        IBGS_HIP(hipGetLastError());
        return 0;
    }
    if (scratch_elems < nblocks + 1) { set_error("scan scratch too small"); return -IBGS_ERR_ALLOC; }
    uint32_t* sums = scratch;
    hipLaunchKernelGGL(scan_chunk_kernel, dim3((unsigned)nblocks), dim3(SCAN_THREADS), 0, s, in, out, n, sums, 0);
    IBGS_HIP(hipGetLastError());
    const size_t used = nblocks + 1 + 32;
    int rc = exclusive_scan_u32(s, sums, sums, nblocks, scratch + used, scratch_elems > used ? scratch_elems - used : 0, true);
    if (rc) return rc;
    hipLaunchKernelGGL(scan_add_kernel, dim3((unsigned)nblocks), dim3(SCAN_THREADS), 0, s, out, n, sums, nblocks, with_total ? 1 : 0);
    IBGS_HIP(hipGetLastError());
    return 0;
}

__device__ __forceinline__ uint32_t wave_rank(uint32_t d, bool valid, int lane, uint64_t lt_mask, uint32_t* wcnt_row, unsigned long long* peer_row)
{
    uint32_t r = 0;
    if (valid) {
        atomicOr(&peer_row[d], 1ull << lane);
        const unsigned long long peers = *reinterpret_cast<volatile unsigned long long*>(&peer_row[d]);
        volatile uint32_t* wc = wcnt_row;
        const uint32_t pre = wc[d];
        r = pre + (uint32_t)__popcll(peers & lt_mask);
        if ((peers & lt_mask) == 0ull) {
            wc[d] = pre + (uint32_t)__popcll(peers);
            *reinterpret_cast<volatile unsigned long long*>(&peer_row[d]) = 0ull;
        }
    }
    return r;
}

template <typename K>
__global__ void __launch_bounds__(RS_THREADS) radix_hist_kernel(const K* __restrict__ keys, size_t n, const uint32_t* __restrict__ n_dev,
                                                                int shift, int nbins, uint32_t* __restrict__ hist, unsigned nblocks)
{
    __shared__ uint32_t h[RS_MAX_BINS];
    if (n_dev) n = min(n, (size_t)*n_dev);
    for (int k = threadIdx.x; k < nbins; k += RS_THREADS) h[k] = 0;
    __syncthreads();
    const size_t base = (size_t)blockIdx.x * RS_CHUNK;
    const uint32_t mask = (uint32_t)nbins - 1;
    const size_t i0 = base + (size_t)threadIdx.x * RS_ITEMS;
    uint32_t kv[RS_ITEMS];
    if (i0 + RS_ITEMS <= n) {
        constexpr int PER = 16 / (int)sizeof(K);
        const uint4* src = reinterpret_cast<const uint4*>(keys + i0);
#pragma unroll
        for (int v = 0; v < RS_ITEMS / PER; v++) {
            const uint4 q = src[v];
            const uint32_t w[4] = {q.x, q.y, q.z, q.w};
#pragma unroll
            for (int e = 0; e < PER; e++)
                kv[v * PER + e] = (sizeof(K) == 4) ? w[e] : ((w[e >> 1] >> ((e & 1) * 16)) & 0xFFFFu);
        }
    } else {
#pragma unroll
        for (int k = 0; k < RS_ITEMS; k++) kv[k] = (i0 + k < n) ? (uint32_t)keys[i0 + k] : 0xFFFFFFFFu;
    }
    const int nvalid = (i0 >= n) ? 0 : (int)((n - i0 < (size_t)RS_ITEMS) ? (n - i0) : (size_t)RS_ITEMS);
    uint32_t run_d = 0, run_n = 0;
#pragma unroll
    for (int k = 0; k < RS_ITEMS; k++) {
        if (k < nvalid) {
            const uint32_t d = (kv[k] >> shift) & mask;
            if (run_n != 0 && d != run_d) { atomicAdd(&h[run_d], run_n); run_n = 0; }
            run_d = d; run_n++;
        }
    }
    if (run_n != 0) atomicAdd(&h[run_d], run_n);
    __syncthreads();
    for (int k = threadIdx.x; k < nbins; k += RS_THREADS) hist[(size_t)k * nblocks + blockIdx.x] = h[k];
}

template <typename K>
__global__ void __launch_bounds__(RS_THREADS) radix_scatter_kernel(const K* __restrict__ keys_in, const uint32_t* __restrict__ vals_in,
                                                                   K* __restrict__ keys_out, uint32_t* __restrict__ vals_out,
                                                                   size_t n, const uint32_t* __restrict__ n_dev, int shift, int nbits, int nbins,
                                                                   const uint32_t* __restrict__ hist_scanned, unsigned nblocks)
{
    __shared__ uint32_t wcnt[4][RS_MAX_BINS];
    if (n_dev) n = min(n, (size_t)*n_dev);
    if ((size_t)blockIdx.x * RS_CHUNK >= n) return;
    __shared__ unsigned long long ptab[4][RS_MAX_BINS];
    __shared__ uint32_t dstart[RS_MAX_BINS];
    __shared__ uint32_t delta[RS_MAX_BINS];
    __shared__ uint32_t lds_wave[4];
    __shared__ uint32_t skey[RS_CHUNK];
    __shared__ uint32_t sval[RS_CHUNK];

    const int lane = threadIdx.x & 63, wave = threadIdx.x >> 6;
    for (int k = threadIdx.x; k < 4 * RS_MAX_BINS; k += RS_THREADS) { (&wcnt[0][0])[k] = 0; (&ptab[0][0])[k] = 0ull; }
    __syncthreads();

    const size_t base = (size_t)blockIdx.x * RS_CHUNK;
    const uint32_t mask = (uint32_t)nbins - 1;
    const uint64_t lt_mask = (lane == 0) ? 0ull : (~0ull >> (64 - lane));

    uint32_t key[RS_ITEMS], val[RS_ITEMS], rank[RS_ITEMS];
#pragma unroll
    for (int k = 0; k < RS_ITEMS; k++) {
        const size_t idx = base + (size_t)wave * (RS_ITEMS * 64) + (size_t)k * 64 + lane;
        const bool valid = idx < n;
        key[k] = valid ? (uint32_t)keys_in[idx] : 0xFFFFFFFFu;
        val[k] = valid ? vals_in[idx] : 0u;
        const uint32_t d = (key[k] >> shift) & mask;
        const uint32_t r = wave_rank(d, valid, lane, lt_mask, &wcnt[wave][0], &ptab[wave][0]);
        rank[k] = r;
    }
    __syncthreads();

    uint32_t tot = 0;
    if (threadIdx.x < nbins) {
        const uint32_t c0 = wcnt[0][threadIdx.x], c1 = wcnt[1][threadIdx.x], c2 = wcnt[2][threadIdx.x], c3 = wcnt[3][threadIdx.x];
        wcnt[0][threadIdx.x] = 0; wcnt[1][threadIdx.x] = c0; wcnt[2][threadIdx.x] = c0 + c1; wcnt[3][threadIdx.x] = c0 + c1 + c2;
        tot = c0 + c1 + c2 + c3;
    }
    uint32_t blocktotal;
    const uint32_t ds = block_exclusive_scan_256(tot, &blocktotal, lds_wave);
    if (threadIdx.x < nbins) {
        dstart[threadIdx.x] = ds;
        delta[threadIdx.x] = hist_scanned[(size_t)threadIdx.x * nblocks + blockIdx.x] - ds;
    }
    __syncthreads();

    const size_t remaining = n - base;
    const uint32_t count = remaining < (size_t)RS_CHUNK ? (uint32_t)remaining : (uint32_t)RS_CHUNK;
#pragma unroll
    for (int k = 0; k < RS_ITEMS; k++) {
        const size_t idx = base + (size_t)wave * (RS_ITEMS * 64) + (size_t)k * 64 + lane;
        if (idx < n) {
            const uint32_t d = (key[k] >> shift) & mask;
            const uint32_t lpos = dstart[d] + wcnt[wave][d] + rank[k];
            skey[lpos] = key[k];
            sval[lpos] = val[k];
        }
    }
    __syncthreads();
#pragma unroll
    for (int k = 0; k < RS_ITEMS; k++) {
        const uint32_t l = (uint32_t)k * RS_THREADS + threadIdx.x;
        if (l < count) {
            const uint32_t kk = skey[l];
            const uint32_t d = (kk >> shift) & mask;
            const uint32_t dst = l + delta[d];
            keys_out[dst] = (K)kk;
            vals_out[dst] = sval[l];
        }
    }
}


constexpr uint32_t OS_FLAG_AGG = 1u << 30, OS_FLAG_INC = 2u << 30, OS_VAL_MASK = (1u << 30) - 1u;
constexpr int OS_MAX_PASS = 4;
constexpr int OS_HIST_THREADS = 1024;
constexpr int OS_THREADS = 512, OS_WAVES = OS_THREADS / 64, OS_ITEMS = RS_CHUNK / OS_THREADS;

__global__ void __launch_bounds__(OS_HIST_THREADS) onesweep_hist_kernel(const uint32_t* __restrict__ keys, size_t n, int npass, int dbits,
                                                                   uint32_t* __restrict__ ghist ,
                                                                   int drop_max , uint32_t* __restrict__ n_kept)
{
    __shared__ uint32_t h[OS_MAX_PASS][RS_MAX_BINS];
    __shared__ uint32_t s_kept;
    for (int k = threadIdx.x; k < OS_MAX_PASS * RS_MAX_BINS; k += OS_HIST_THREADS) (&h[0][0])[k] = 0;
    if (threadIdx.x == 0) s_kept = 0;
    __syncthreads();
    const uint32_t mask = (1u << dbits) - 1u;
    const size_t stride = (size_t)gridDim.x * OS_HIST_THREADS;
    uint32_t kept = 0;
    for (size_t i = (size_t)blockIdx.x * OS_HIST_THREADS + threadIdx.x; i < n; i += stride) {
        const uint32_t k = keys[i];
        if (drop_max && k == 0xFFFFFFFFu) continue;
        kept++;
        for (int p = 0; p < npass; p++) atomicAdd(&h[p][(k >> (p * dbits)) & mask], 1u);
    }
    if (kept) atomicAdd(&s_kept, kept);
    __syncthreads();
    if (threadIdx.x == 0 && s_kept) atomicAdd(n_kept, s_kept);
    for (int k = threadIdx.x; k < npass * RS_MAX_BINS; k += OS_HIST_THREADS) {
        const uint32_t c = (&h[0][0])[k];
        if (c) atomicAdd(&ghist[k], c);
    }
}

__global__ void __launch_bounds__(OS_THREADS) onesweep_pass_kernel(const uint32_t* __restrict__ keys_in, const uint32_t* __restrict__ vals_in,
                                                                   uint32_t* __restrict__ keys_out, uint32_t* __restrict__ vals_out,
                                                                   size_t n, int shift, int nbits, int nbins,
                                                                   const uint32_t* __restrict__ ghist ,
                                                                   uint32_t* __restrict__ status ,
                                                                   uint32_t* __restrict__ ticket, uint32_t* __restrict__ err,
                                                                   int drop_here ,
                                                                   const uint32_t* __restrict__ n_kept ,
                                                                   uint32_t* __restrict__ stays ,
                                                                   uint32_t spin_limit )
{
    __shared__ uint32_t wcnt[OS_WAVES][RS_MAX_BINS];
    __shared__ unsigned long long ptab[OS_WAVES][RS_MAX_BINS];
    __shared__ uint32_t dstart[RS_MAX_BINS];
    __shared__ uint32_t delta[RS_MAX_BINS];
    __shared__ uint32_t lds_wave[4];
    __shared__ uint32_t skey[RS_CHUNK];
    __shared__ uint32_t sval[RS_CHUNK];
    __shared__ uint32_t s_bid;

    const int lane = threadIdx.x & 63, wave = threadIdx.x >> 6;
    const uint32_t kept = *n_kept;
    const size_t n_in = drop_here ? n : (size_t)kept;
    if (threadIdx.x == 0) s_bid = atomicAdd(ticket, 1u);
    for (int k = threadIdx.x; k < OS_WAVES * RS_MAX_BINS; k += OS_THREADS) { (&wcnt[0][0])[k] = 0; (&ptab[0][0])[k] = 0ull; }
    __syncthreads();
    const uint32_t bid = s_bid;
    const size_t base = (size_t)bid * RS_CHUNK;
    if (base >= n_in) return;

    const int all_one_bin = __syncthreads_or((int)(threadIdx.x < (unsigned)nbins && kept != 0u && ghist[threadIdx.x] == kept));
    if (all_one_bin && (!drop_here || (size_t)kept == n)) {
        if (stays) { if (bid == 0 && threadIdx.x == 0) *stays = 1u; return; }
#pragma unroll
        for (int k = 0; k < OS_ITEMS; k++) {
            const size_t idx = base + (size_t)k * OS_THREADS + threadIdx.x;
            if (idx < n_in) { keys_out[idx] = keys_in[idx]; vals_out[idx] = vals_in[idx]; }
        }
        return;
    }

    const uint32_t mask = (uint32_t)nbins - 1;
    const uint64_t lt_mask = (lane == 0) ? 0ull : (~0ull >> (64 - lane));

    uint32_t key[OS_ITEMS], val[OS_ITEMS], rank[OS_ITEMS];
    uint32_t takes = 0;
#pragma unroll
    for (int k = 0; k < OS_ITEMS; k++) {
        const size_t idx = base + (size_t)wave * (OS_ITEMS * 64) + (size_t)k * 64 + lane;
        const bool inside = idx < n_in;
        key[k] = inside ? keys_in[idx] : 0xFFFFFFFFu;
        val[k] = inside ? vals_in[idx] : 0u;
        const bool valid = inside && !(drop_here && key[k] == 0xFFFFFFFFu);
        takes |= valid ? (1u << k) : 0u;
        const uint32_t d = (key[k] >> shift) & mask;
        const uint32_t r = wave_rank(d, valid, lane, lt_mask, &wcnt[wave][0], &ptab[wave][0]);
        rank[k] = r;
    }
    __syncthreads();

    uint32_t tot = 0;
    if (threadIdx.x < nbins) {
#pragma unroll
        for (int w = 0; w < OS_WAVES; w++) { const uint32_t c = wcnt[w][threadIdx.x]; wcnt[w][threadIdx.x] = tot; tot += c; }
        uint32_t* mine = status + (size_t)bid * RS_MAX_BINS + threadIdx.x;
        __hip_atomic_store(mine, (bid == 0 ? OS_FLAG_INC : OS_FLAG_AGG) | tot, __ATOMIC_RELAXED, __HIP_MEMORY_SCOPE_AGENT);
    }
    uint32_t gtotal, ltotal;
    const uint32_t gstart = block_exclusive_scan_256(threadIdx.x < nbins ? ghist[threadIdx.x] : 0u, &gtotal, lds_wave);
    const uint32_t ds = block_exclusive_scan_256(tot, &ltotal, lds_wave);
    if (spin_limit == 0u && bid == 0 && threadIdx.x == 0) *err = 1u;
    if (threadIdx.x < nbins) {
        uint32_t excl = 0;
        if (bid > 0) {
            constexpr int LOOKBACK = 8;
            int64_t b = (int64_t)bid - 1;
            uint32_t spins = 0;
            bool done = false;
            while (!done && b >= 0) {
                uint32_t st[LOOKBACK];
#pragma unroll
                for (int k = 0; k < LOOKBACK; k++)
                    st[k] = (b - k >= 0) ? __hip_atomic_load(status + (size_t)(b - k) * RS_MAX_BINS + threadIdx.x, __ATOMIC_RELAXED, __HIP_MEMORY_SCOPE_AGENT)
                                         : OS_FLAG_INC;
                int used = 0;
#pragma unroll
                for (int k = 0; k < LOOKBACK; k++) {
                    if (done || used != k) continue;
                    const uint32_t flag = st[k] & ~OS_VAL_MASK;
                    if (flag == 0u) continue;
                    excl += st[k] & OS_VAL_MASK;
                    used = k + 1;
                    if (flag == OS_FLAG_INC) done = true;
                }
                b -= used;
                if (!done && used < LOOKBACK) {
                    if (++spins > (spin_limit ? spin_limit : (1u << 26))) { *err = 1u; break; }
                    __builtin_amdgcn_s_sleep(1);
                }
            }
            __hip_atomic_store(status + (size_t)bid * RS_MAX_BINS + threadIdx.x, OS_FLAG_INC | ((excl + tot) & OS_VAL_MASK),
                               __ATOMIC_RELAXED, __HIP_MEMORY_SCOPE_AGENT);
        }
        dstart[threadIdx.x] = ds;
        delta[threadIdx.x] = gstart + excl - ds;
    }
    __syncthreads();

    const uint32_t count = ltotal;
#pragma unroll
    for (int k = 0; k < OS_ITEMS; k++) {
        if (takes & (1u << k)) {
            const uint32_t d = (key[k] >> shift) & mask;
            const uint32_t lpos = dstart[d] + wcnt[wave][d] + rank[k];
            skey[lpos] = key[k];
            sval[lpos] = val[k];
        }
    }
    __syncthreads();
#pragma unroll
    for (int k = 0; k < OS_ITEMS; k++) {
        const uint32_t l = (uint32_t)k * OS_THREADS + threadIdx.x;
        if (l < count) {
            const uint32_t kk = skey[l];
            const uint32_t d = (kk >> shift) & mask;
            const uint32_t dst = l + delta[d];
            keys_out[dst] = kk;
            vals_out[dst] = sval[l];
        }
    }
}

static int g_use_onesweep = getenv("IBGS_RADIX_ONESWEEP") ? atoi(getenv("IBGS_RADIX_ONESWEEP")) : -1;
static uint32_t g_lookback_spins = 1u << 26;
void radix_set_onesweep(bool on) { g_use_onesweep = on ? 1 : 0; }
void radix_set_lookback_spins(uint32_t v) { g_lookback_spins = v; }
constexpr size_t OS_AUTO_MAX_CHUNKS = 4096;

static size_t onesweep_elems(size_t n)
{
    const size_t nblocks = (n + RS_CHUNK - 1) / RS_CHUNK;
    return (size_t)OS_MAX_PASS * RS_MAX_BINS + 64 + (size_t)OS_MAX_PASS * (nblocks ? nblocks : 1) * RS_MAX_BINS;
}

static int radix_sort_pairs_onesweep(hipStream_t s, uint32_t* keys[2], uint32_t* vals[2], size_t n, int npass, int dbits,
                                     uint32_t* scratch, size_t scratch_elems, uint32_t* err_dev, uint32_t* kept_dev, bool scratch_is_zero, uint32_t* result_alt)
{
    const unsigned nblocks = (unsigned)((n + RS_CHUNK - 1) / RS_CHUNK);
    const int nbins = 1 << dbits;
    const size_t need = (size_t)OS_MAX_PASS * RS_MAX_BINS + 64 + (size_t)npass * nblocks * RS_MAX_BINS;
    if (scratch_elems < need) { set_error("onesweep scratch too small"); return -IBGS_ERR_ALLOC; }
    uint32_t* ghist = scratch;
    uint32_t* tickets = scratch + OS_MAX_PASS * RS_MAX_BINS;
    uint32_t* status = tickets + 64;
    if (!scratch_is_zero) IBGS_HIP(hipMemsetAsync(scratch, 0, need * sizeof(uint32_t), s));
    const unsigned hb = (unsigned)((n + 8u * OS_HIST_THREADS - 1) / (8u * OS_HIST_THREADS));
    const unsigned hblocks = hb < 256u ? (hb ? hb : 1u) : 256u;
    hipLaunchKernelGGL(onesweep_hist_kernel, dim3(hblocks), dim3(OS_HIST_THREADS), 0, s, keys[0], n, npass, dbits, ghist, kept_dev ? 1 : 0, kept_dev ? kept_dev : tickets + 33);
    IBGS_HIP(hipGetLastError());
    int cur = 0;
    for (int pass = 0; pass < npass; pass++) {
        hipLaunchKernelGGL(onesweep_pass_kernel, dim3(nblocks), dim3(OS_THREADS), 0, s, keys[cur], vals[cur], keys[cur ^ 1], vals[cur ^ 1],
                           n, pass * dbits, dbits, nbins, ghist + pass * RS_MAX_BINS, status + (size_t)pass * nblocks * RS_MAX_BINS,
                           tickets + pass, err_dev ? err_dev : tickets + 32, (kept_dev && pass == 0) ? 1 : 0, kept_dev ? kept_dev : tickets + 33,
                           (result_alt && npass == 4 && pass == 3) ? result_alt : (uint32_t*)nullptr, g_lookback_spins);
        IBGS_HIP(hipGetLastError());
        cur ^= 1;
    }
    if (cur != 0) {
        IBGS_HIP(hipMemcpyAsync(keys[0], keys[1], n * sizeof(uint32_t), hipMemcpyDeviceToDevice, s));
        IBGS_HIP(hipMemcpyAsync(vals[0], vals[1], n * sizeof(uint32_t), hipMemcpyDeviceToDevice, s));
    }
    if (!err_dev) {
        uint32_t flag = 0;
        IBGS_HIP(hipMemcpyAsync(&flag, tickets + 32, sizeof(flag), hipMemcpyDeviceToHost, s));
        IBGS_HIP(hipStreamSynchronize(s));
        if (flag) { set_error("radix sort: a decoupled look-back timed out (result discarded)"); return -IBGS_ERR_HIP; }
    }
    return 0;
}

size_t radix_hist_elems(size_t n)
{
    const size_t nblocks = (n + RS_CHUNK - 1) / RS_CHUNK;
    const size_t hist = (size_t)RS_MAX_BINS * (nblocks ? nblocks : 1) + 1;
    const size_t classic = hist + 64 + scan_scratch_elems(hist);
    const size_t os = onesweep_elems(n);
    return classic > os ? classic : os;
}

__global__ void __launch_bounds__(RS_THREADS) count_kept_kernel(const uint32_t* __restrict__ keys, size_t n, uint32_t* __restrict__ kept)
{
    uint32_t c = 0;
    for (size_t i = (size_t)blockIdx.x * RS_THREADS + threadIdx.x; i < n; i += (size_t)gridDim.x * RS_THREADS) c += keys[i] != 0xFFFFFFFFu ? 1u : 0u;
    for (int d = 32; d >= 1; d >>= 1) c += (uint32_t)__shfl_xor((int)c, d, 64);
    if ((threadIdx.x & 63) == 0 && c) atomicAdd(kept, c);
}

size_t radix_zero_elems(size_t n, int nbits_total)
{
    if (n == 0 || nbits_total <= 0) return 0;
    const size_t nblocks = (n + RS_CHUNK - 1) / RS_CHUNK;
    const int npass = (nbits_total + 7) / 8;
    const bool want_os = g_use_onesweep >= 0 ? g_use_onesweep != 0 : nblocks <= OS_AUTO_MAX_CHUNKS;
    if (!(want_os && npass <= OS_MAX_PASS && n < (size_t)OS_VAL_MASK)) return 0;
    return (size_t)OS_MAX_PASS * RS_MAX_BINS + 64 + (size_t)npass * nblocks * RS_MAX_BINS;
}

int radix_sort_pairs(hipStream_t s, uint32_t* keys[2], uint32_t* vals[2], size_t n, int nbits_total,
                     uint32_t* hist, size_t hist_elems, uint32_t* err_dev, uint32_t* kept_dev, bool scratch_is_zero, uint32_t* result_alt)
{
    if (n == 0 || nbits_total <= 0) return 0;
    const unsigned nblocks = (unsigned)((n + RS_CHUNK - 1) / RS_CHUNK);
    const int npass = (nbits_total + 7) / 8;
    const int dbits = (nbits_total + npass - 1) / npass;
    const int nbins = 1 << dbits;
    const bool want_os = g_use_onesweep >= 0 ? g_use_onesweep != 0 : nblocks <= OS_AUTO_MAX_CHUNKS;
    if (want_os && npass <= OS_MAX_PASS && n < (size_t)OS_VAL_MASK)
        return radix_sort_pairs_onesweep(s, keys, vals, n, npass, dbits, hist, hist_elems, err_dev, kept_dev, scratch_is_zero, result_alt);
    const size_t hist_n = (size_t)nbins * nblocks;
    if (hist_elems < hist_n + 1 + 64) { set_error("radix scratch too small"); return -IBGS_ERR_ALLOC; }
    uint32_t* scan_scratch = hist + hist_n + 1 + 63;
    const size_t scan_elems = hist_elems - (hist_n + 1 + 63);
    if (kept_dev) {
        hipLaunchKernelGGL(count_kept_kernel, dim3(nblocks < 1024u ? nblocks : 1024u), dim3(RS_THREADS), 0, s, keys[0], n, kept_dev);
        IBGS_HIP(hipGetLastError());
    }
    int cur = 0;
    for (int pass = 0; pass < npass; pass++) {
        const int shift = pass * dbits;
        hipLaunchKernelGGL(radix_hist_kernel<uint32_t>, dim3(nblocks), dim3(RS_THREADS), 0, s, keys[cur], n, (const uint32_t*)nullptr, shift, nbins, hist, nblocks);
        IBGS_HIP(hipGetLastError());
        int rc = exclusive_scan_u32(s, hist, hist, hist_n, scan_scratch, scan_elems, false);
        if (rc) return rc;
        hipLaunchKernelGGL(radix_scatter_kernel<uint32_t>, dim3(nblocks), dim3(RS_THREADS), 0, s, keys[cur], vals[cur], keys[cur ^ 1], vals[cur ^ 1],
                           n, (const uint32_t*)nullptr, shift, dbits, nbins, hist, nblocks);
        IBGS_HIP(hipGetLastError());
        cur ^= 1;
    }
    if (cur != 0) {
        IBGS_HIP(hipMemcpyAsync(keys[0], keys[1], n * sizeof(uint32_t), hipMemcpyDeviceToDevice, s));
        IBGS_HIP(hipMemcpyAsync(vals[0], vals[1], n * sizeof(uint32_t), hipMemcpyDeviceToDevice, s));
    }
    return 0;
}

}
```

Measured before the change: 571.7.

## Fuse SH color evaluation into the onesweep radix sort launches

The spherical-harmonics color pass and the rendered-note signal no longer run as a separate kernel after preprocess. When the onesweep path is taken, that work rides inside the depth-sort kernels. The per-wave SH color code moves into a shared header so both the preprocess and sort translation units can call it. The aim is to remove a kernel launch and overlap the SH memory traffic with sort work, at the cost of heavier sort kernels with more registers and LDS pressure, and tighter coupling between the stages.

Measured after the change: 583.5, median of 6. 1.02x the previous value.

```diff
diff --git a/ibgs_amd/_build.py b/ibgs_amd/_build.py
--- a/ibgs_amd/_build.py
+++ b/ibgs_amd/_build.py
@@ -10,6 +10,7 @@
 SOURCES = ["api", "preprocess", "scan_sort", "binning", "render_fwd", "render_bwd", "preprocess_bwd", "knn", "adam", "compact", "deterministic", "loss", "depth_normal", "activate"]
 EXTRA = {
     "preprocess": ["-ffp-contract=off"],
+    "scan_sort": ["-ffp-contract=off"],
     "render_fwd": ["-fno-slp-vectorize"],
     "render_bwd": ["-fno-slp-vectorize", "-fno-signed-zeros"],
 }
diff --git a/ibgs_amd/csrc/api.hip b/ibgs_amd/csrc/api.hip
--- a/ibgs_amd/csrc/api.hip
+++ b/ibgs_amd/csrc/api.hip
@@ -1,4 +1,5 @@
 #include "common.h"
+#include "sh_color.h"
 #include <sched.h>
 #include <time.h>
 #include <string.h>
@@ -273,6 +274,7 @@
     out[0] = g_last_stats[0]; out[1] = g_last_stats[1]; out[2] = g_last_stats[2];
 }
 void ibgs_debug_set_lookback_spins(uint32_t v) { radix_set_lookback_spins(v); }
+void ibgs_debug_set_sh_ride(int32_t on) { radix_set_sh_ride(on != 0); }
 int32_t ibgs_check_async(void* stream, int32_t wait)
 {
     hipStream_t s = reinterpret_cast<hipStream_t>(stream);
@@ -349,19 +351,24 @@
     RSlot* rs = rslot(s, true);
     if (!rs) return -IBGS_ERR_HIP;
     uint32_t ticket = 0;
+    ShRide ride;
+    bool riding = false;
     { StageTimer t(s, IBGS_STAGE_PREPROCESS);
       if ((rc = launch_preprocess(s, a, g, deferred ? 1 : 0))) return rc;
       if (deferred) {
           ticket = ++rs->seq;
           const RenderedNote note{g.tile_partial, (uint32_t)nwaves, ticket, rs->host};
-          if ((rc = launch_preprocess(s, a, g, 2, &note)) < 0) return rc;
-          if (rc == 0) { hipLaunchKernelGGL(rendered_note_kernel, dim3(1), dim3(1024), 0, s, note); IBGS_HIP(hipGetLastError()); }
+          riding = radix_takes_sh_ride((size_t)Pn, 32) && preprocess_sh_ride(a, g, &note, &ride);
+          if (!riding) {
+              if ((rc = launch_preprocess(s, a, g, 2, &note)) < 0) return rc;
+              if (rc == 0) { hipLaunchKernelGGL(rendered_note_kernel, dim3(1), dim3(1024), 0, s, note); IBGS_HIP(hipGetLastError()); }
+          }
       }
     }
     if ((rc = stage_check(s, debug, "preprocess"))) return rc;
     { StageTimer t(s, IBGS_STAGE_DEPTH_SORT);
       if ((rc = radix_sort_pairs(s, g.sort_key, g.sort_val, (size_t)Pn, 32, g.hist, g.hist_elems, deferred ? g.tile_partial + nwaves : g.offsets + Pn + 1,
-                                 g.offsets + Pn + 3, true, g.offsets + Pn + 4))) return rc; }
+                                 g.offsets + Pn + 3, true, g.offsets + Pn + 4, riding ? &ride : nullptr))) return rc; }
     if ((rc = stage_check(s, debug, "depth sort"))) return rc;
     { StageTimer t(s, IBGS_STAGE_SCAN);
       if (!deferred && (rc = exclusive_scan_u32(s, g.tiles, g.offsets, (size_t)Pn, g.hist, g.hist_elems, true))) return rc; }
diff --git a/ibgs_amd/csrc/common.h b/ibgs_amd/csrc/common.h
--- a/ibgs_amd/csrc/common.h
+++ b/ibgs_amd/csrc/common.h
@@ -335,13 +335,17 @@
         __hip_atomic_store(n.host + 2, n.ticket, __ATOMIC_RELEASE, __HIP_MEMORY_SCOPE_SYSTEM);
     }
 }
+struct ShRide;
 int launch_preprocess(hipStream_t s, const ibgs_forward_args& a, const GeomState& g, int phase = 0, const RenderedNote* note = nullptr);
+bool preprocess_sh_ride(const ibgs_forward_args& a, const GeomState& g, const RenderedNote* note, ShRide* out);
 int launch_mark_visible(hipStream_t s, int P, const float* means3D, const float* vm, uint8_t* present);
 
 size_t radix_hist_elems(size_t n);
 int radix_sort_pairs(hipStream_t s, uint32_t* keys[2], uint32_t* vals[2], size_t n, int nbits,
                      uint32_t* hist, size_t hist_elems, uint32_t* err_dev = nullptr, uint32_t* kept_dev = nullptr, bool scratch_is_zero = false,
-                     uint32_t* result_alt = nullptr);
+                     uint32_t* result_alt = nullptr, const ShRide* ride = nullptr);
+bool radix_takes_sh_ride(size_t n, int nbits);
+void radix_set_sh_ride(bool on);
 size_t radix_zero_elems(size_t n, int nbits);
 int exclusive_scan_u32(hipStream_t s, const uint32_t* in, uint32_t* out, size_t n, uint32_t* scratch,
                        size_t scratch_elems, bool with_total);
diff --git a/ibgs_amd/csrc/preprocess.hip b/ibgs_amd/csrc/preprocess.hip
--- a/ibgs_amd/csrc/preprocess.hip
+++ b/ibgs_amd/csrc/preprocess.hip
@@ -1,35 +1,8 @@
 #include "common.h"
+#include "sh_color.h"
 #include <stdlib.h>
 
 namespace ibgs {
-
-__constant__ float kC0 = 0.28209479177387814f;
-__constant__ float kC1 = 0.4886025119029199f;
-__constant__ float kC2[5] = {1.0925484305920792f, -1.0925484305920792f, 0.31539156525252005f,
-                             -1.0925484305920792f, 0.5462742152960396f};
-__constant__ float kC3[7] = {-0.5900435899266435f, 2.890611442640554f, -0.4570457994644658f,
-                             0.3731763325901154f, -0.4570457994644658f, 1.445305721320277f,
-                             -0.5900435899266435f};
-
-struct PreParams {
-    int P, D, M;
-    const float* means3D; const float* scales; const float* rotations; const float* opacities;
-    const float* shs; const float* shs_rest;
-    const float* cov3D_precomp; const float* colors_precomp; const float* all_map;
-    const float* plane_normal; const float* plane_offset; int plane_mode;
-    int inst0;
-    int tile_row0;
-    float scale_modifier;
-    int depth_only;
-    int32_t* radii;
-    float* rec; float* depths; float* cov3D; uint32_t* tiles; uint4* fp; uint64_t* tmask_hi; uint8_t* clamped;
-    uint64_t* alive64;
-    uint32_t* sort_key; uint32_t* sort_val;
-    int cull;
-    uint32_t* zero_a; uint32_t zero_a_n; uint32_t* zero_b; uint32_t zero_b_n;
-    RenderedNote note;
-    uint32_t* tile_partial; int partial0; int partial_err;
-};
 
 __device__ __forceinline__ float ndc_to_pix(float v, int S)
 {
@@ -407,140 +380,15 @@
     p.sort_val[o] = (uint32_t)o;
 }
 
-constexpr int SHC_ROW = 52;
 template <bool SPLIT>
 __global__ void __launch_bounds__(256) sh_color_kernel(PreParams p, Cam cam)
 {
-    __shared__ float s_sh_all[4][32 * SHC_ROW];
+    __shared__ float s_sh_all[4][SHC_WAVE_FLOATS];
     if (p.note.host != nullptr && blockIdx.x == 0) {
         __shared__ unsigned long long s_note[4];
         rendered_note_block<256>(p.note, s_note);
     }
-    float* s_sh = s_sh_all[threadIdx.x >> 6];
-    const int lane = threadIdx.x & 63;
-    const int wave = blockIdx.x * 4 + (threadIdx.x >> 6);
-    const int first = wave * 64;
-    if (first >= p.P) return;
-    const uint64_t alive_m = p.alive64[wave];
-    if (alive_m == 0ull) return;
-    const int i = min(first + lane, p.P - 1);
-    const bool alive = (alive_m >> lane) & 1ull;
-    const int D = p.D, M = p.M;
-    const int nb = (D + 1) * (D + 1);
-    const float px3 = p.means3D[3 * i], py3 = p.means3D[3 * i + 1], pz3 = p.means3D[3 * i + 2];
-    float shv[48];
-    if (SPLIT && M == 16 && first + 64 <= p.P) {
-        const float4* rest4 = reinterpret_cast<const float4*>(p.shs_rest + (size_t)first * 45);
-        const float4* dc4 = reinterpret_cast<const float4*>(p.shs + (size_t)first * 3);
-        float4 v[12];
-#pragma unroll
-        for (int it = 0; it < 12; it++) {
-            const int h = it / 6, qp = (it % 6) * 64 + lane;
-            if (qp < 360) {
-                const int ra = (4 * qp) / 45, rb = (4 * qp + 3) / 45;
-                const bool need = nb > 1 && (((alive_m >> (32 * h + ra)) & 1ull) || ((alive_m >> (32 * h + rb)) & 1ull));
-                v[it] = need ? rest4[360 * h + qp] : make_float4(0.f, 0.f, 0.f, 0.f);
-            } else {
-                const int ra = (4 * (qp - 360)) / 3, rb = (4 * (qp - 360) + 3) / 3;
-                const bool need = (((alive_m >> (32 * h + ra)) & 3ull) != 0ull) || ((alive_m >> (32 * h + rb)) & 1ull);
-                v[it] = need ? dc4[24 * h + (qp - 360)] : make_float4(0.f, 0.f, 0.f, 0.f);
-            }
-        }
-        float4* s_raw = reinterpret_cast<float4*>(s_sh);
-#pragma unroll
-        for (int h = 0; h < 2; h++) {
-#pragma unroll
-            for (int it = 0; it < 6; it++) s_raw[it * 64 + lane] = v[h * 6 + it];
-            if ((lane >> 5) == h) {
-                const float* rr = s_sh + 45 * (lane & 31);
-                const float* rd = s_sh + 1440 + 3 * (lane & 31);
-                shv[0] = rd[0]; shv[1] = rd[1]; shv[2] = rd[2];
-#pragma unroll
-                for (int k = 0; k < 45; k++) shv[3 + k] = rr[k];
-            }
-        }
-    } else if (SPLIT) {
-        const float* sr = p.shs_rest + (size_t)i * (M - 1) * 3;
-        const float* sd = p.shs + (size_t)i * 3;
-#pragma unroll
-        for (int k = 0; k < 48; k++) shv[k] = (alive && k < 3 * nb) ? (k < 3 ? sd[k] : sr[k - 3]) : 0.f;
-    } else if (M == 16) {
-        const float4* src = reinterpret_cast<const float4*>(p.shs) + (size_t)first * 12;
-        const int nq = min(64, p.P - first) * 12;
-        float4 v[12];
-#pragma unroll
-        for (int it = 0; it < 12; it++) {
-            const int q = it * 64 + lane;
-            const int row = q / 12, piece = q - row * 12;
-            const bool ok = q < nq && ((alive_m >> row) & 1ull) && 4 * piece < 3 * nb;
-            v[it] = ok ? src[q] : make_float4(0.f, 0.f, 0.f, 0.f);
-        }
-#pragma unroll
-        for (int h = 0; h < 2; h++) {
-#pragma unroll
-            for (int it = 0; it < 6; it++) {
-                const int q = it * 64 + lane;
-                const int row = q / 12, piece = q - row * 12;
-                *reinterpret_cast<float4*>(s_sh + row * SHC_ROW + piece * 4) = v[h * 6 + it];
-            }
-            if ((lane >> 5) == h) {
-                const float4* row4 = reinterpret_cast<const float4*>(s_sh + (lane & 31) * SHC_ROW);
-#pragma unroll
-                for (int k = 0; k < 12; k++) { const float4 q = row4[k]; shv[4 * k] = q.x; shv[4 * k + 1] = q.y; shv[4 * k + 2] = q.z; shv[4 * k + 3] = q.w; }
-            }
-        }
-    } else {
-        const float* sh = p.shs + (size_t)i * M * 3;
-#pragma unroll
-        for (int k = 0; k < 48; k++) shv[k] = (alive && k < 3 * nb) ? sh[k] : 0.f;
-    }
-    if (!alive) return;
-    float d0 = px3 - cam.campos[0], d1 = py3 - cam.campos[1], d2 = pz3 - cam.campos[2];
-    const float len = sqrtf(d0 * d0 + d1 * d1 + d2 * d2);
-    d0 /= len; d1 /= len; d2 /= len;
-    float B[16];
-    B[0] = kC0;
-    if (D > 0) {
-        const float x = d0, y = d1, z = d2;
-        B[1] = -kC1 * y; B[2] = kC1 * z; B[3] = -kC1 * x;
-        if (D > 1) {
-            const float xx = x * x, yy = y * y, zz = z * z, xy = x * y, yz = y * z, xz = x * z;
-            B[4] = kC2[0] * xy; B[5] = kC2[1] * yz; B[6] = kC2[2] * (2.0f * zz - xx - yy);
-            B[7] = kC2[3] * xz; B[8] = kC2[4] * (xx - yy);
-            if (D > 2) {
-                B[9] = kC3[0] * y * (3.0f * xx - yy);
-                B[10] = kC3[1] * xy * z;
-                B[11] = kC3[2] * y * (4.0f * zz - xx - yy);
-                B[12] = kC3[3] * z * (2.0f * zz - 3.0f * xx - 3.0f * yy);
-                B[13] = kC3[4] * x * (4.0f * zz - xx - yy);
-                B[14] = kC3[5] * z * (xx - yy);
-                B[15] = kC3[6] * x * (xx - 3.0f * yy);
-            }
-        }
-    }
-    float col[3];
-#pragma unroll
-    for (int ch = 0; ch < 3; ch++) col[ch] = B[0] * shv[ch];
-#pragma unroll
-    for (int k = 1; k < 16; k++) {
-        if (k < nb) {
-#pragma unroll
-            for (int ch = 0; ch < 3; ch++) col[ch] = col[ch] + B[k] * shv[3 * k + ch];
-        }
-    }
-    const int o = p.inst0 + i;
-    uint8_t clampbits = 0;
-    float4 out;
-    float* oc = &out.x;
-#pragma unroll
-    for (int ch = 0; ch < 3; ch++) {
-        const float v = col[ch] + 0.5f;
-        if (v < 0) clampbits |= (uint8_t)(1u << ch);
-        oc[ch] = fmaxf(v, 0.0f);
-    }
-    out.w = 0.f;
-    reinterpret_cast<float4*>(p.rec)[(size_t)o * 4 + 2] = out;
-    p.clamped[o] = clampbits;
+    sh_color_wave<SPLIT>(p, cam, blockIdx.x * 4 + (threadIdx.x >> 6), s_sh_all[threadIdx.x >> 6]);
 }
 
 __global__ void __launch_bounds__(256) mark_visible_kernel(int P, const float* means3D, Cam cam, uint8_t* present)
@@ -556,11 +404,10 @@
     return a.shs && !a.colors_precomp && !a.render_depth_only;
 }
 
-int launch_preprocess(hipStream_t s, const ibgs_forward_args& a, const GeomState& g, int phase, const RenderedNote* note)
-{
-    PreParams p;
+static PreParams make_params(const ibgs_forward_args& a, const GeomState& g)
+{
+    PreParams p{};
     p.note = RenderedNote{nullptr, 0u, 0u, nullptr};
-    int carried = 0;
     p.P = a.P; p.D = a.D; p.M = a.M;
     p.means3D = a.means3D; p.scales = a.scales; p.rotations = a.rotations; p.opacities = a.opacities;
     p.shs = a.shs; p.shs_rest = a.shs_rest; p.cov3D_precomp = a.cov3D_precomp; p.colors_precomp = a.colors_precomp; p.all_map = a.all_map;
@@ -569,6 +416,26 @@
     p.radii = a.radii; p.rec = g.rec; p.depths = g.depths; p.cov3D = g.cov3D; p.tiles = g.tiles; p.fp = g.fp; p.tmask_hi = g.tmask_hi;
     p.clamped = g.clamped; p.sort_key = g.sort_key[0]; p.sort_val = g.sort_val[0];
     p.cull = !(a.flags & IBGS_FLAG_NO_TILE_CULL) && !(a.render_depth_only && a.buffer_length == 1);
+    return p;
+}
+
+bool preprocess_sh_ride(const ibgs_forward_args& a, const GeomState& g, const RenderedNote* note, ShRide* out)
+{
+    if (!preprocess_is_split(a) || a.n_views > 1) return false;
+    out->p = make_params(a, g);
+    out->p.inst0 = 0; out->p.tile_row0 = 0;
+    out->p.alive64 = g.alive64;
+    if (note) out->p.note = *note;
+    out->cam = make_cam(a.viewmatrix, a.projmatrix, a.campos, a.bg, a.tanfovx, a.tanfovy, a.W, a.H);
+    out->split = a.shs_rest != nullptr;
+    out->waves = (a.P + 63) / 64;
+    return true;
+}
+
+int launch_preprocess(hipStream_t s, const ibgs_forward_args& a, const GeomState& g, int phase, const RenderedNote* note)
+{
+    PreParams p = make_params(a, g);
+    int carried = 0;
     const int blocks = (a.P + 255) / 256;
     const int nv = a.n_views > 1 ? a.n_views : 1;
     const int gy = (a.H + TILE - 1) / TILE;
diff --git a/ibgs_amd/csrc/scan_sort.hip b/ibgs_amd/csrc/scan_sort.hip
--- a/ibgs_amd/csrc/scan_sort.hip
+++ b/ibgs_amd/csrc/scan_sort.hip
@@ -1,4 +1,5 @@
 #include "common.h"
+#include "sh_color.h"
 #include <cstdlib>
 
 namespace ibgs {
@@ -251,52 +252,64 @@
 constexpr int OS_HIST_THREADS = 1024;
 constexpr int OS_THREADS = 512, OS_WAVES = OS_THREADS / 64, OS_ITEMS = RS_CHUNK / OS_THREADS;
 
-__global__ void __launch_bounds__(OS_HIST_THREADS) onesweep_hist_kernel(const uint32_t* __restrict__ keys, size_t n, int npass, int dbits,
-                                                                   uint32_t* __restrict__ ghist ,
-                                                                   int drop_max , uint32_t* __restrict__ n_kept)
-{
-    __shared__ uint32_t h[OS_MAX_PASS][RS_MAX_BINS];
-    __shared__ uint32_t s_kept;
-    for (int k = threadIdx.x; k < OS_MAX_PASS * RS_MAX_BINS; k += OS_HIST_THREADS) (&h[0][0])[k] = 0;
-    if (threadIdx.x == 0) s_kept = 0;
+template <int NT>
+__device__ __forceinline__ void onesweep_hist_block(const uint32_t* __restrict__ keys, size_t n, int npass, int dbits, uint32_t* __restrict__ ghist,
+                                                    int drop_max, uint32_t* __restrict__ n_kept, unsigned nblk, uint32_t (*h)[RS_MAX_BINS], uint32_t* s_kept)
+{
+    for (int k = threadIdx.x; k < OS_MAX_PASS * RS_MAX_BINS; k += NT) (&h[0][0])[k] = 0;
+    if (threadIdx.x == 0) *s_kept = 0;
     __syncthreads();
     const uint32_t mask = (1u << dbits) - 1u;
-    const size_t stride = (size_t)gridDim.x * OS_HIST_THREADS;
+    const size_t stride = (size_t)nblk * NT;
     uint32_t kept = 0;
-    for (size_t i = (size_t)blockIdx.x * OS_HIST_THREADS + threadIdx.x; i < n; i += stride) {
+    for (size_t i = (size_t)blockIdx.x * NT + threadIdx.x; i < n; i += stride) {
         const uint32_t k = keys[i];
         if (drop_max && k == 0xFFFFFFFFu) continue;
         kept++;
         for (int p = 0; p < npass; p++) atomicAdd(&h[p][(k >> (p * dbits)) & mask], 1u);
     }
-    if (kept) atomicAdd(&s_kept, kept);
-    __syncthreads();
-    if (threadIdx.x == 0 && s_kept) atomicAdd(n_kept, s_kept);
-    for (int k = threadIdx.x; k < npass * RS_MAX_BINS; k += OS_HIST_THREADS) {
+    if (kept) atomicAdd(s_kept, kept);
+    __syncthreads();
+    if (threadIdx.x == 0 && *s_kept) atomicAdd(n_kept, *s_kept);
+    for (int k = threadIdx.x; k < npass * RS_MAX_BINS; k += NT) {
         const uint32_t c = (&h[0][0])[k];
         if (c) atomicAdd(&ghist[k], c);
     }
 }
 
-__global__ void __launch_bounds__(OS_THREADS) onesweep_pass_kernel(const uint32_t* __restrict__ keys_in, const uint32_t* __restrict__ vals_in,
-                                                                   uint32_t* __restrict__ keys_out, uint32_t* __restrict__ vals_out,
-                                                                   size_t n, int shift, int nbits, int nbins,
-                                                                   const uint32_t* __restrict__ ghist ,
-                                                                   uint32_t* __restrict__ status ,
-                                                                   uint32_t* __restrict__ ticket, uint32_t* __restrict__ err,
-                                                                   int drop_here ,
-                                                                   const uint32_t* __restrict__ n_kept ,
-                                                                   uint32_t* __restrict__ stays ,
-                                                                   uint32_t spin_limit )
-{
-    __shared__ uint32_t wcnt[OS_WAVES][RS_MAX_BINS];
-    __shared__ unsigned long long ptab[OS_WAVES][RS_MAX_BINS];
-    __shared__ uint32_t dstart[RS_MAX_BINS];
-    __shared__ uint32_t delta[RS_MAX_BINS];
-    __shared__ uint32_t lds_wave[4];
-    __shared__ uint32_t skey[RS_CHUNK];
-    __shared__ uint32_t sval[RS_CHUNK];
-    __shared__ uint32_t s_bid;
+__global__ void __launch_bounds__(OS_HIST_THREADS) onesweep_hist_kernel(const uint32_t* __restrict__ keys, size_t n, int npass, int dbits,
+                                                                   uint32_t* __restrict__ ghist ,
+                                                                   int drop_max , uint32_t* __restrict__ n_kept)
+{
+    __shared__ uint32_t h[OS_MAX_PASS][RS_MAX_BINS];
+    __shared__ uint32_t s_kept;
+    onesweep_hist_block<OS_HIST_THREADS>(keys, n, npass, dbits, ghist, drop_max, n_kept, gridDim.x, h, &s_kept);
+}
+
+struct OsPassLds {
+    unsigned long long ptab[OS_WAVES][RS_MAX_BINS];
+    uint32_t wcnt[OS_WAVES][RS_MAX_BINS];
+    uint32_t dstart[RS_MAX_BINS];
+    uint32_t delta[RS_MAX_BINS];
+    uint32_t lds_wave[4];
+    uint32_t skey[RS_CHUNK];
+    uint32_t sval[RS_CHUNK];
+    uint32_t s_bid;
+};
+
+__device__ __forceinline__ void onesweep_pass_block(const uint32_t* __restrict__ keys_in, const uint32_t* __restrict__ vals_in,
+                                                   uint32_t* __restrict__ keys_out, uint32_t* __restrict__ vals_out,
+                                                   size_t n, int shift, int nbits, int nbins,
+                                                   const uint32_t* __restrict__ ghist ,
+                                                   uint32_t* __restrict__ status ,
+                                                   uint32_t* __restrict__ ticket, uint32_t* __restrict__ err,
+                                                   int drop_here ,
+                                                   const uint32_t* __restrict__ n_kept ,
+                                                   uint32_t* __restrict__ stays ,
+                                                   uint32_t spin_limit ,
+                                                   OsPassLds& L)
+{
+    auto& wcnt = L.wcnt; auto& ptab = L.ptab; auto& dstart = L.dstart; auto& delta = L.delta; auto& lds_wave = L.lds_wave; auto& skey = L.skey; auto& sval = L.sval; auto& s_bid = L.s_bid;
 
     const int lane = threadIdx.x & 63, wave = threadIdx.x >> 6;
     const uint32_t kept = *n_kept;
@@ -410,8 +423,83 @@
     }
 }
 
+__global__ void __launch_bounds__(OS_THREADS) onesweep_pass_kernel(const uint32_t* __restrict__ keys_in, const uint32_t* __restrict__ vals_in,
+                                                                   uint32_t* __restrict__ keys_out, uint32_t* __restrict__ vals_out,
+                                                                   size_t n, int shift, int nbits, int nbins,
+                                                                   const uint32_t* __restrict__ ghist ,
+                                                                   uint32_t* __restrict__ status ,
+                                                                   uint32_t* __restrict__ ticket, uint32_t* __restrict__ err,
+                                                                   int drop_here ,
+                                                                   const uint32_t* __restrict__ n_kept ,
+                                                                   uint32_t* __restrict__ stays ,
+                                                                   uint32_t spin_limit )
+{
+    __shared__ OsPassLds L;
+    onesweep_pass_block(keys_in, vals_in, keys_out, vals_out, n, shift, nbits, nbins, ghist, status, ticket, err, drop_here, n_kept, stays, spin_limit, L);
+}
+
+constexpr int OS_HIST_WAVES = OS_HIST_THREADS / 64;
+union OsHistShLds {
+    struct { uint32_t h[OS_MAX_PASS][RS_MAX_BINS]; uint32_t kept; } hist;
+    float sh[OS_HIST_WAVES][SHC_WAVE_FLOATS];
+};
+union OsPassShLds {
+    OsPassLds sort;
+    float sh[OS_WAVES][SHC_WAVE_FLOATS];
+};
+
+template <bool SPLIT, int WAVES >
+__device__ __forceinline__ void sh_ride_block(const ShRide& r, unsigned j , int wave0, int wave1, float (*sh)[SHC_WAVE_FLOATS])
+{
+    const int wave = wave0 + (int)j * WAVES + (int)(threadIdx.x >> 6);
+    if (wave < wave1) sh_color_wave<SPLIT>(r.p, r.cam, wave, sh[threadIdx.x >> 6]);
+}
+
+template <bool SPLIT>
+__global__ void __launch_bounds__(OS_HIST_THREADS) onesweep_hist_sh_kernel(const uint32_t* __restrict__ keys, size_t n, int npass, int dbits, uint32_t* __restrict__ ghist,
+                                                                      int drop_max, uint32_t* __restrict__ n_kept, unsigned nhist, ShRide r, int wave0, int wave1)
+{
+    __shared__ OsHistShLds L;
+    if (blockIdx.x < nhist) { onesweep_hist_block<OS_HIST_THREADS>(keys, n, npass, dbits, ghist, drop_max, n_kept, nhist, L.hist.h, &L.hist.kept); return; }
+    const unsigned j = blockIdx.x - nhist;
+    if (j == 0 && r.p.note.host != nullptr) {
+        __shared__ unsigned long long s_note[OS_HIST_WAVES];
+        rendered_note_block<OS_HIST_THREADS>(r.p.note, s_note);
+    }
+    sh_ride_block<SPLIT, OS_HIST_WAVES>(r, j, wave0, wave1, L.sh);
+}
+
+template <bool SPLIT>
+__global__ void __launch_bounds__(OS_THREADS) onesweep_pass_sh_kernel(const uint32_t* __restrict__ keys_in, const uint32_t* __restrict__ vals_in,
+                                                                      uint32_t* __restrict__ keys_out, uint32_t* __restrict__ vals_out,
+                                                                      size_t n, int shift, int nbits, int nbins, const uint32_t* __restrict__ ghist,
+                                                                      uint32_t* __restrict__ status, uint32_t* __restrict__ ticket, uint32_t* __restrict__ err,
+                                                                      int drop_here, const uint32_t* __restrict__ n_kept, uint32_t* __restrict__ stays, uint32_t spin_limit,
+                                                                      unsigned nsort, ShRide r, int wave0, int wave1)
+{
+    __shared__ OsPassShLds L;
+    if (blockIdx.x >= nsort) { sh_ride_block<SPLIT, OS_WAVES>(r, blockIdx.x - nsort, wave0, wave1, L.sh); return; }
+    onesweep_pass_block(keys_in, vals_in, keys_out, vals_out, n, shift, nbits, nbins, ghist, status, ticket, err, drop_here, n_kept, stays, spin_limit, L.sort);
+}
+
 static int g_use_onesweep = getenv("IBGS_RADIX_ONESWEEP") ? atoi(getenv("IBGS_RADIX_ONESWEEP")) : -1;
 static uint32_t g_lookback_spins = 1u << 26;
+static int g_sh_ride_w[1 + OS_MAX_PASS] = {5, 18, 18, 18, 0};
+static int g_sh_ride = [] {
+    const char* e = getenv("IBGS_SH_RIDE");
+    if (!e) return 1;
+    int w[1 + OS_MAX_PASS] = {0, 0, 0, 0, 0}, k = 0, sum = 0;
+    for (const char* c = e; *c && k <= OS_MAX_PASS; k++) {
+        w[k] = atoi(c);
+        sum += w[k] > 0 ? w[k] : 0;
+        while (*c && *c != ',') c++;
+        if (*c == ',') c++;
+    }
+    if (sum <= 0) return 0;
+    for (int i = 0; i <= OS_MAX_PASS; i++) g_sh_ride_w[i] = w[i] > 0 ? w[i] : 0;
+    return 1;
+}();
+void radix_set_sh_ride(bool on) { g_sh_ride = on ? 1 : 0; }
 void radix_set_onesweep(bool on) { g_use_onesweep = on ? 1 : 0; }
 void radix_set_lookback_spins(uint32_t v) { g_lookback_spins = v; }
 constexpr size_t OS_AUTO_MAX_CHUNKS = 4096;
@@ -423,7 +511,8 @@
 }
 
 static int radix_sort_pairs_onesweep(hipStream_t s, uint32_t* keys[2], uint32_t* vals[2], size_t n, int npass, int dbits,
-                                     uint32_t* scratch, size_t scratch_elems, uint32_t* err_dev, uint32_t* kept_dev, bool scratch_is_zero, uint32_t* result_alt)
+                                     uint32_t* scratch, size_t scratch_elems, uint32_t* err_dev, uint32_t* kept_dev, bool scratch_is_zero, uint32_t* result_alt,
+                                     const ShRide* ride)
 {
     const unsigned nblocks = (unsigned)((n + RS_CHUNK - 1) / RS_CHUNK);
     const int nbins = 1 << dbits;
@@ -433,16 +522,46 @@
     uint32_t* tickets = scratch + OS_MAX_PASS * RS_MAX_BINS;
     uint32_t* status = tickets + 64;
     if (!scratch_is_zero) IBGS_HIP(hipMemsetAsync(scratch, 0, need * sizeof(uint32_t), s));
+    int cut[2 + OS_MAX_PASS] = {0, 0, 0, 0, 0, 0};
+    if (ride) {
+        int wsum = 0;
+        for (int k = 0; k <= npass; k++) wsum += g_sh_ride_w[k];
+        if (wsum <= 0) { set_error("SH ride without weights"); return -IBGS_ERR_INVALID; }
+        int acc = 0;
+        for (int k = 0; k <= npass; k++) { acc += g_sh_ride_w[k]; cut[k + 1] = (int)((int64_t)ride->waves * acc / wsum); }
+    }
+    auto sh_groups = [&](int k, int waves) { return (unsigned)((cut[k + 1] - cut[k] + waves - 1) / waves); };
+    const uint32_t* kept_arg = kept_dev ? kept_dev : tickets + 33;
     const unsigned hb = (unsigned)((n + 8u * OS_HIST_THREADS - 1) / (8u * OS_HIST_THREADS));
     const unsigned hblocks = hb < 256u ? (hb ? hb : 1u) : 256u;
-    hipLaunchKernelGGL(onesweep_hist_kernel, dim3(hblocks), dim3(OS_HIST_THREADS), 0, s, keys[0], n, npass, dbits, ghist, kept_dev ? 1 : 0, kept_dev ? kept_dev : tickets + 33);
+    if (!ride) {
+        hipLaunchKernelGGL(onesweep_hist_kernel, dim3(hblocks), dim3(OS_HIST_THREADS), 0, s, keys[0], n, npass, dbits, ghist, kept_dev ? 1 : 0, kept_dev ? kept_dev : tickets + 33);
+    } else {
+        unsigned g = sh_groups(0, OS_HIST_WAVES);
+        if (g == 0 && ride->p.note.host) g = 1;
+        const dim3 grid(hblocks + g);
+        if (ride->split) hipLaunchKernelGGL(onesweep_hist_sh_kernel<true>, grid, dim3(OS_HIST_THREADS), 0, s, keys[0], n, npass, dbits, ghist, kept_dev ? 1 : 0, kept_dev ? kept_dev : tickets + 33, hblocks, *ride, cut[0], cut[1]);
+        else hipLaunchKernelGGL(onesweep_hist_sh_kernel<false>, grid, dim3(OS_HIST_THREADS), 0, s, keys[0], n, npass, dbits, ghist, kept_dev ? 1 : 0, kept_dev ? kept_dev : tickets + 33, hblocks, *ride, cut[0], cut[1]);
+    }
     IBGS_HIP(hipGetLastError());
     int cur = 0;
     for (int pass = 0; pass < npass; pass++) {
-        hipLaunchKernelGGL(onesweep_pass_kernel, dim3(nblocks), dim3(OS_THREADS), 0, s, keys[cur], vals[cur], keys[cur ^ 1], vals[cur ^ 1],
-                           n, pass * dbits, dbits, nbins, ghist + pass * RS_MAX_BINS, status + (size_t)pass * nblocks * RS_MAX_BINS,
-                           tickets + pass, err_dev ? err_dev : tickets + 32, (kept_dev && pass == 0) ? 1 : 0, kept_dev ? kept_dev : tickets + 33,
-                           (result_alt && npass == 4 && pass == 3) ? result_alt : (uint32_t*)nullptr, g_lookback_spins);
+        uint32_t* st = status + (size_t)pass * nblocks * RS_MAX_BINS;
+        uint32_t* e = err_dev ? err_dev : tickets + 32;
+        const int drop = (kept_dev && pass == 0) ? 1 : 0;
+        uint32_t* stays = (result_alt && npass == 4 && pass == 3) ? result_alt : (uint32_t*)nullptr;
+        const unsigned g = ride ? sh_groups(1 + pass, OS_WAVES) : 0u;
+        if (g == 0)
+            hipLaunchKernelGGL(onesweep_pass_kernel, dim3(nblocks), dim3(OS_THREADS), 0, s, keys[cur], vals[cur], keys[cur ^ 1], vals[cur ^ 1],
+                               n, pass * dbits, dbits, nbins, ghist + pass * RS_MAX_BINS, st, tickets + pass, e, drop, kept_arg, stays, g_lookback_spins);
+        else if (ride->split)
+            hipLaunchKernelGGL(onesweep_pass_sh_kernel<true>, dim3(nblocks + g), dim3(OS_THREADS), 0, s, keys[cur], vals[cur], keys[cur ^ 1], vals[cur ^ 1],
+                               n, pass * dbits, dbits, nbins, ghist + pass * RS_MAX_BINS, st, tickets + pass, e, drop, kept_arg, stays, g_lookback_spins,
+                               nblocks, *ride, cut[1 + pass], cut[2 + pass]);
+        else
+            hipLaunchKernelGGL(onesweep_pass_sh_kernel<false>, dim3(nblocks + g), dim3(OS_THREADS), 0, s, keys[cur], vals[cur], keys[cur ^ 1], vals[cur ^ 1],
+                               n, pass * dbits, dbits, nbins, ghist + pass * RS_MAX_BINS, st, tickets + pass, e, drop, kept_arg, stays, g_lookback_spins,
+                               nblocks, *ride, cut[1 + pass], cut[2 + pass]);
         IBGS_HIP(hipGetLastError());
         cur ^= 1;
     }
@@ -486,8 +605,17 @@
     return (size_t)OS_MAX_PASS * RS_MAX_BINS + 64 + (size_t)npass * nblocks * RS_MAX_BINS;
 }
 
+bool radix_takes_sh_ride(size_t n, int nbits_total)
+{
+    if (!g_sh_ride || n == 0 || nbits_total <= 0) return false;
+    const size_t nblocks = (n + RS_CHUNK - 1) / RS_CHUNK;
+    const int npass = (nbits_total + 7) / 8;
+    const bool want_os = g_use_onesweep >= 0 ? g_use_onesweep != 0 : nblocks <= OS_AUTO_MAX_CHUNKS;
+    return want_os && npass <= OS_MAX_PASS && n < (size_t)OS_VAL_MASK;
+}
+
 int radix_sort_pairs(hipStream_t s, uint32_t* keys[2], uint32_t* vals[2], size_t n, int nbits_total,
-                     uint32_t* hist, size_t hist_elems, uint32_t* err_dev, uint32_t* kept_dev, bool scratch_is_zero, uint32_t* result_alt)
+                     uint32_t* hist, size_t hist_elems, uint32_t* err_dev, uint32_t* kept_dev, bool scratch_is_zero, uint32_t* result_alt, const ShRide* ride)
 {
     if (n == 0 || nbits_total <= 0) return 0;
     const unsigned nblocks = (unsigned)((n + RS_CHUNK - 1) / RS_CHUNK);
@@ -496,7 +624,8 @@
     const int nbins = 1 << dbits;
     const bool want_os = g_use_onesweep >= 0 ? g_use_onesweep != 0 : nblocks <= OS_AUTO_MAX_CHUNKS;
     if (want_os && npass <= OS_MAX_PASS && n < (size_t)OS_VAL_MASK)
-        return radix_sort_pairs_onesweep(s, keys, vals, n, npass, dbits, hist, hist_elems, err_dev, kept_dev, scratch_is_zero, result_alt);
+        return radix_sort_pairs_onesweep(s, keys, vals, n, npass, dbits, hist, hist_elems, err_dev, kept_dev, scratch_is_zero, result_alt, ride);
+    if (ride) { set_error("radix sort: an SH ride needs the single-launch passes (radix_takes_sh_ride)"); return -IBGS_ERR_INVALID; }
     const size_t hist_n = (size_t)nbins * nblocks;
     if (hist_elems < hist_n + 1 + 64) { set_error("radix scratch too small"); return -IBGS_ERR_ALLOC; }
     uint32_t* scan_scratch = hist + hist_n + 1 + 63;
diff --git a/ibgs_amd/csrc/sh_color.h b/ibgs_amd/csrc/sh_color.h
--- /dev/null
+++ b/ibgs_amd/csrc/sh_color.h
@@ -0,0 +1,172 @@
+#pragma once
+#include "common.h"
+
+namespace ibgs {
+
+static __constant__ float kC0 = 0.28209479177387814f;
+static __constant__ float kC1 = 0.4886025119029199f;
+static __constant__ float kC2[5] = {1.0925484305920792f, -1.0925484305920792f, 0.31539156525252005f,
+                                    -1.0925484305920792f, 0.5462742152960396f};
+static __constant__ float kC3[7] = {-0.5900435899266435f, 2.890611442640554f, -0.4570457994644658f,
+                                    0.3731763325901154f, -0.4570457994644658f, 1.445305721320277f,
+                                    -0.5900435899266435f};
+
+struct PreParams {
+    int P, D, M;
+    const float* means3D; const float* scales; const float* rotations; const float* opacities;
+    const float* shs; const float* shs_rest;
+    const float* cov3D_precomp; const float* colors_precomp; const float* all_map;
+    const float* plane_normal; const float* plane_offset; int plane_mode;
+    int inst0;
+    int tile_row0;
+    float scale_modifier;
+    int depth_only;
+    int32_t* radii;
+    float* rec; float* depths; float* cov3D; uint32_t* tiles; uint4* fp; uint64_t* tmask_hi; uint8_t* clamped;
+    uint64_t* alive64;
+    uint32_t* sort_key; uint32_t* sort_val;
+    int cull;
+    uint32_t* zero_a; uint32_t zero_a_n; uint32_t* zero_b; uint32_t zero_b_n;
+    RenderedNote note;
+    uint32_t* tile_partial; int partial0; int partial_err;
+};
+
+constexpr int SHC_ROW = 52;
+constexpr int SHC_WAVE_FLOATS = 32 * SHC_ROW;
+template <bool SPLIT>
+__device__ __forceinline__ void sh_color_wave(const PreParams& p, const Cam& cam, int wave, float* s_sh)
+{
+    const int lane = threadIdx.x & 63;
+    const int first = wave * 64;
+    if (first >= p.P) return;
+    const uint64_t alive_m = p.alive64[wave];
+    if (alive_m == 0ull) return;
+    const int i = min(first + lane, p.P - 1);
+    const bool alive = (alive_m >> lane) & 1ull;
+    const int D = p.D, M = p.M;
+    const int nb = (D + 1) * (D + 1);
+    const float px3 = p.means3D[3 * i], py3 = p.means3D[3 * i + 1], pz3 = p.means3D[3 * i + 2];
+    float shv[48];
+    if (SPLIT && M == 16 && first + 64 <= p.P) {
+        const float4* rest4 = reinterpret_cast<const float4*>(p.shs_rest + (size_t)first * 45);
+        const float4* dc4 = reinterpret_cast<const float4*>(p.shs + (size_t)first * 3);
+        float4 v[12];
+#pragma unroll
+        for (int it = 0; it < 12; it++) {
+            const int h = it / 6, qp = (it % 6) * 64 + lane;
+            if (qp < 360) {
+                const int ra = (4 * qp) / 45, rb = (4 * qp + 3) / 45;
+                const bool need = nb > 1 && (((alive_m >> (32 * h + ra)) & 1ull) || ((alive_m >> (32 * h + rb)) & 1ull));
+                v[it] = need ? rest4[360 * h + qp] : make_float4(0.f, 0.f, 0.f, 0.f);
+            } else {
+                const int ra = (4 * (qp - 360)) / 3, rb = (4 * (qp - 360) + 3) / 3;
+                const bool need = (((alive_m >> (32 * h + ra)) & 3ull) != 0ull) || ((alive_m >> (32 * h + rb)) & 1ull);
+                v[it] = need ? dc4[24 * h + (qp - 360)] : make_float4(0.f, 0.f, 0.f, 0.f);
+            }
+        }
+        float4* s_raw = reinterpret_cast<float4*>(s_sh);
+#pragma unroll
+        for (int h = 0; h < 2; h++) {
+#pragma unroll
+            for (int it = 0; it < 6; it++) s_raw[it * 64 + lane] = v[h * 6 + it];
+            if ((lane >> 5) == h) {
+                const float* rr = s_sh + 45 * (lane & 31);
+                const float* rd = s_sh + 1440 + 3 * (lane & 31);
+                shv[0] = rd[0]; shv[1] = rd[1]; shv[2] = rd[2];
+#pragma unroll
+                for (int k = 0; k < 45; k++) shv[3 + k] = rr[k];
+            }
+        }
+    } else if (SPLIT) {
+        const float* sr = p.shs_rest + (size_t)i * (M - 1) * 3;
+        const float* sd = p.shs + (size_t)i * 3;
+#pragma unroll
+        for (int k = 0; k < 48; k++) shv[k] = (alive && k < 3 * nb) ? (k < 3 ? sd[k] : sr[k - 3]) : 0.f;
+    } else if (M == 16) {
+        const float4* src = reinterpret_cast<const float4*>(p.shs) + (size_t)first * 12;
+        const int nq = min(64, p.P - first) * 12;
+        float4 v[12];
+#pragma unroll
+        for (int it = 0; it < 12; it++) {
+            const int q = it * 64 + lane;
+            const int row = q / 12, piece = q - row * 12;
+            const bool ok = q < nq && ((alive_m >> row) & 1ull) && 4 * piece < 3 * nb;
+            v[it] = ok ? src[q] : make_float4(0.f, 0.f, 0.f, 0.f);
+        }
+#pragma unroll
+        for (int h = 0; h < 2; h++) {
+#pragma unroll
+            for (int it = 0; it < 6; it++) {
+                const int q = it * 64 + lane;
+                const int row = q / 12, piece = q - row * 12;
+                *reinterpret_cast<float4*>(s_sh + row * SHC_ROW + piece * 4) = v[h * 6 + it];
+            }
+            if ((lane >> 5) == h) {
+                const float4* row4 = reinterpret_cast<const float4*>(s_sh + (lane & 31) * SHC_ROW);
+#pragma unroll
+                for (int k = 0; k < 12; k++) { const float4 q = row4[k]; shv[4 * k] = q.x; shv[4 * k + 1] = q.y; shv[4 * k + 2] = q.z; shv[4 * k + 3] = q.w; }
+            }
+        }
+    } else {
+        const float* sh = p.shs + (size_t)i * M * 3;
+#pragma unroll
+        for (int k = 0; k < 48; k++) shv[k] = (alive && k < 3 * nb) ? sh[k] : 0.f;
+    }
+    if (!alive) return;
+    float d0 = px3 - cam.campos[0], d1 = py3 - cam.campos[1], d2 = pz3 - cam.campos[2];
+    const float len = sqrtf(d0 * d0 + d1 * d1 + d2 * d2);
+    d0 /= len; d1 /= len; d2 /= len;
+    float B[16];
+    B[0] = kC0;
+    if (D > 0) {
+        const float x = d0, y = d1, z = d2;
+        B[1] = -kC1 * y; B[2] = kC1 * z; B[3] = -kC1 * x;
+        if (D > 1) {
+            const float xx = x * x, yy = y * y, zz = z * z, xy = x * y, yz = y * z, xz = x * z;
+            B[4] = kC2[0] * xy; B[5] = kC2[1] * yz; B[6] = kC2[2] * (2.0f * zz - xx - yy);
+            B[7] = kC2[3] * xz; B[8] = kC2[4] * (xx - yy);
+            if (D > 2) {
+                B[9] = kC3[0] * y * (3.0f * xx - yy);
+                B[10] = kC3[1] * xy * z;
+                B[11] = kC3[2] * y * (4.0f * zz - xx - yy);
+                B[12] = kC3[3] * z * (2.0f * zz - 3.0f * xx - 3.0f * yy);
+                B[13] = kC3[4] * x * (4.0f * zz - xx - yy);
+                B[14] = kC3[5] * z * (xx - yy);
+                B[15] = kC3[6] * x * (xx - 3.0f * yy);
+            }
+        }
+    }
+    float col[3];
+#pragma unroll
+    for (int ch = 0; ch < 3; ch++) col[ch] = B[0] * shv[ch];
+#pragma unroll
+    for (int k = 1; k < 16; k++) {
+        if (k < nb) {
+#pragma unroll
+            for (int ch = 0; ch < 3; ch++) col[ch] = col[ch] + B[k] * shv[3 * k + ch];
+        }
+    }
+    const int o = p.inst0 + i;
+    uint8_t clampbits = 0;
+    float4 out;
+    float* oc = &out.x;
+#pragma unroll
+    for (int ch = 0; ch < 3; ch++) {
+        const float v = col[ch] + 0.5f;
+        if (v < 0) clampbits |= (uint8_t)(1u << ch);
+        oc[ch] = fmaxf(v, 0.0f);
+    }
+    out.w = 0.f;
+    reinterpret_cast<float4*>(p.rec)[(size_t)o * 4 + 2] = out;
+    p.clamped[o] = clampbits;
+}
+
+
+struct ShRide {
+    PreParams p;
+    Cam cam;
+    int split;
+    int waves;
+};
+
+}
```
